# xhuan8/SoccerPlayerShapePose

Hardware: NVIDIA B200
Metric: SMPL meshes/sec fwd+bwd (higher is better)
Workload: dtype f32 (bf16x3 split on tcgen05, fp32 accumulate)

## Files before the change

### soccerplayershapepose_b200/csrc/api.cu

```cuda
#include <atomic>
#include <cstring>
#include <map>
#include <mutex>

#include <nvtx3/nvToolsExt.h>

#include "common.cuh"
#include "umma_common.cuh"

namespace b200smpl {

bool pdl_enabled() {
  static const bool on = getenv("B200_PDL") == nullptr || atoi(getenv("B200_PDL")) != 0;
  return on;
}

NvtxRange::NvtxRange(const char* name) { nvtxRangePushA(name); }
NvtxRange::~NvtxRange() { nvtxRangePop(); }

static thread_local std::string g_last_error;
static std::atomic<long long> g_launches{0};

void set_error(const std::string& msg) { g_last_error = msg; }
int fail(int code, const std::string& msg) {
  g_last_error = msg;
  return code;
}
void count_launch(int n) { g_launches.fetch_add(n, std::memory_order_relaxed); }

static std::atomic<int> g_timing{0};
static std::mutex g_timing_mu;
struct TimingRec { const char* name; cudaEvent_t a, b; };
static std::vector<TimingRec> g_timing_recs;

LaunchTimer::LaunchTimer(const char* name, cudaStream_t st) : name_(name), st_(st), nvtx_(name) {
  if (g_timing.load(std::memory_order_relaxed)) {
    if (cudaEventCreate(&start_) == cudaSuccess) cudaEventRecord(start_, st_);
    else start_ = nullptr;
  }
}
LaunchTimer::~LaunchTimer() {
  if (start_ == nullptr) return;
  cudaEvent_t stop = nullptr;
  if (cudaEventCreate(&stop) != cudaSuccess) return;
  cudaEventRecord(stop, st_);
  std::lock_guard<std::mutex> lk(g_timing_mu);
  g_timing_recs.push_back({name_, start_, stop});
}

static int fwd_gemm_mode(int mode) { return mode == B200SMPL_MODE_BF16_FAST ? B200SMPL_MODE_BF16 : mode; }
static int bwd_gemm_mode(int mode) {
  return mode == B200SMPL_MODE_BF16 ? B200SMPL_MODE_FP32 : (mode == B200SMPL_MODE_BF16_FAST ? B200SMPL_MODE_BF16 : mode);
}

constexpr int DEFAULT_SLAB = 4096;
constexpr int MAX_SLAB = 40960;
static_assert(MAX_SLAB == 2 * BM * BS_MAX_WORK, "slab cap = the forward GEMMs' work-list capacity");
constexpr int MIN_SLABS_PER_SPLIT = 4;

struct Plan {
  int S;
  int k_splits;
  size_t off_feat, off_featf, off_A, off_jposed, off_vpT;
  size_t off_dvp_hi, off_dvp_lo, off_dA, off_dtr, off_dJtot, off_dfeat;
  size_t total;
  size_t saved_slab_bytes;
};

static size_t align_up(size_t x, size_t a) { return (x + a - 1) / a * a; }

static Plan make_plan(const b200smpl_model* m, int batch, int mode, int slab_bodies, bool backward) {
  const DevModel& d = m->dm;
  Plan p{};
  const int Bp = round_up(std::max(batch, 1), 128);
  const int S = slab_bodies > 0 ? round_up(std::min(slab_bodies, MAX_SLAB), 128) : DEFAULT_SLAB;
  p.S = std::min(S, Bp);
  size_t off = 0;
  auto take = [&](size_t bytes) {
    const size_t o = off;
    off = align_up(off + bytes, 1024);
    return o;
  };
  const size_t S_ = (size_t)p.S;
  p.off_feat = take(S_ * d.fl.pitch * 2);
  p.off_featf = take(mode == B200SMPL_MODE_FP32_SIMT ? S_ * d.fl.nf_pad * 4 : 0);
  p.off_A = take((size_t)NJ * AELEMS * S_ * 4);
  p.off_jposed = take((size_t)NJ * 3 * S_ * 4);
  p.off_vpT = take((size_t)d.n_pad * S_ * 4);
  p.saved_slab_bytes = align_up((size_t)NJ * AELEMS * S_ * 4, 1024) + align_up((size_t)d.n_pad * S_ * 4, 1024);
  if (backward) {
    const int bmode = bwd_gemm_mode(mode);
    p.k_splits = bmode == B200SMPL_MODE_FP32_SIMT ? 1 : blend_bwd_umma_splits(d, p.S, m->num_sms);
    p.off_dvp_hi = take(S_ * d.n_pad * 2);
    p.off_dvp_lo = take(bmode == B200SMPL_MODE_BF16 ? 0 : S_ * d.n_pad * 2);
    p.off_dA = take((size_t)(NJ * AELEMS + 3) * S_ * 4);
    p.off_dtr = p.off_dA + (size_t)NJ * AELEMS * S_ * 4;
    p.off_dJtot = take((size_t)std::max(batch, 1) * d.njout * 3 * 4);
    p.off_dfeat = take((size_t)p.k_splits * S_ * d.fl.nf_pad * 4);
  }
  p.total = off + 1024;
  return p;
}

static int check_common(const b200smpl_model* m, int batch, int mode, const void* ws) {
  if (m == nullptr) return fail(B200SMPL_ERR_INVALID, "null model handle");
  if (m->device < 0) return fail(B200SMPL_ERR_CUDA, "host-only model handle: no CUDA device (there is no CPU fallback)");
  if (batch < 1) return fail(B200SMPL_ERR_INVALID, "batch must be >= 1");
  if (mode != B200SMPL_MODE_FP32 && mode != B200SMPL_MODE_BF16 && mode != B200SMPL_MODE_FP32_SIMT &&
      mode != B200SMPL_MODE_BF16_FAST)
    return fail(B200SMPL_ERR_INVALID, "unknown mode");
  if (ws == nullptr) return fail(B200SMPL_ERR_WORKSPACE, "null workspace");
  return 0;
}

}

using namespace b200smpl;

extern "C" {

int b200smpl_abi_version(void) { return B200SMPL_ABI_VERSION; }
const char* b200smpl_last_error(void) { return g_last_error.c_str(); }
int64_t b200smpl_launch_count(void) { return (int64_t)g_launches.load(); }

void b200smpl_timing_enable(int enable) { g_timing.store(enable ? 1 : 0); }

size_t b200smpl_timing_report(char* buf, size_t cap) {
  std::vector<TimingRec> recs;
  {
    std::lock_guard<std::mutex> lk(g_timing_mu);
    recs.swap(g_timing_recs);
  }
  std::map<std::string, std::pair<long long, double>> agg;
  for (auto& r : recs) {
    float ms = 0.f;
    if (cudaEventSynchronize(r.b) == cudaSuccess && cudaEventElapsedTime(&ms, r.a, r.b) == cudaSuccess) {
      auto& e = agg[r.name];
      e.first += 1;
      e.second += ms;
    }
    cudaEventDestroy(r.a);
    cudaEventDestroy(r.b);
  }
  std::string out;
  for (auto& kv : agg) out += kv.first + " " + std::to_string(kv.second.first) + " " + std::to_string(kv.second.second) + "\n";
  if (buf != nullptr && cap > 0) {
    const size_t n = std::min(cap - 1, out.size());
    memcpy(buf, out.data(), n);
    buf[n] = 0;
  }
  return out.size() + 1;
}

int b200smpl_model_create(const b200smpl_model_desc* desc, int device, b200smpl_model** out) {
  B200_NVTX("b200smpl_model_create");
  if (desc == nullptr || out == nullptr) return fail(B200SMPL_ERR_INVALID, "null argument");
  *out = nullptr;
  b200smpl_model* m = new b200smpl_model();
  std::string err;
  int rc = pack_model(desc, m->host, m->dm, err);
  if (rc != 0) {
    delete m;
    return fail(rc, err);
  }
  m->nvj = desc->num_vertex_joints;
  m->nreg = desc->num_regressed_joints;
  m->device = device;
  if (device < 0) {
    *out = m;
    return 0;
  }
  auto cleanup = [&]() {
    for (void* p : m->allocs) cudaFree(p);
    delete m;
  };
  int prev = 0;
  cudaError_t e = cudaGetDevice(&prev);
  if (e == cudaSuccess) e = cudaSetDevice(device);
  if (e != cudaSuccess) {
    cleanup();
    return fail(B200SMPL_ERR_CUDA, std::string("cudaSetDevice: ") + cudaGetErrorString(e));
  }
  cudaDeviceProp prop;
  if (cudaGetDeviceProperties(&prop, device) == cudaSuccess) {
    m->num_sms = prop.multiProcessorCount;
    if (prop.major != 10) {
      cleanup();
      cudaSetDevice(prev);
      return fail(B200SMPL_ERR_CUDA, "this library is built for sm_100a (B200) only; device is sm_" +
                                         std::to_string(prop.major) + std::to_string(prop.minor));
    }
  }
  auto upload = [&](const void* src, size_t bytes, const void** dst) -> bool {
    void* p = nullptr;
    if (cudaMalloc(&p, std::max<size_t>(bytes, 16)) != cudaSuccess) return false;
    m->allocs.push_back(p);
    if (bytes && cudaMemcpy(p, src, bytes, cudaMemcpyHostToDevice) != cudaSuccess) return false;
    *dst = p;
    return true;
  };
  HostArrays& h = m->host;
  DevModel& d = m->dm;
  bool ok = true;
#define UP(field, vec) ok = ok && upload((vec).data(), (vec).size() * sizeof((vec)[0]), (const void**)&d.field)
  UP(Wf, h.Wf);
  UP(Wb_hi, h.Wb_hi);
  UP(Wb_lo, h.Wb_lo);
  UP(W32, h.W32);
  UP(vmeta, h.vmeta);
  UP(vwts, h.vwts);
  UP(vplan, h.vplan);
  UP(Jt, h.Jt);
  UP(Jsd, h.Jsd);
  UP(term_ptr, h.term_ptr);
  UP(term_joint, h.term_joint);
  UP(term_qrow, h.term_qrow);
  UP(term_c, h.term_c);
  UP(qmeta, h.qmeta);
  UP(qcoef, h.qcoef);
  UP(vt_j0, h.vt_j0);
  UP(vt_nj, h.vt_nj);
#undef UP
  cudaSetDevice(prev);
  if (!ok) {
    e = cudaGetLastError();
    cleanup();
    return fail(B200SMPL_ERR_CUDA, std::string("model upload failed: ") + cudaGetErrorString(e));
  }
  *out = m;
  return 0;
}

void b200smpl_model_destroy(b200smpl_model* m) {
  if (m == nullptr) return;
  for (void* p : m->allocs) cudaFree(p);
  delete m;
}

int b200smpl_model_get_info(const b200smpl_model* m, b200smpl_model_info* info) {
  if (m == nullptr || info == nullptr) return fail(B200SMPL_ERR_INVALID, "null argument");
  info->num_verts = m->dm.V;
  info->num_joints_out = m->dm.njout;
  info->num_betas = m->dm.fl.nb;
  info->num_blend_rows = m->dm.n_rows;
  info->num_blend_rows_padded = m->dm.n_pad;
  info->feature_pitch = m->dm.fl.pitch;
  info->num_virtual_groups = m->dm.nq;
  info->device = m->device;
  return 0;
}

int b200smpl_model_debug_array(const b200smpl_model* m, const char* name, const void** data, size_t* bytes) {
  if (m == nullptr || name == nullptr || data == nullptr || bytes == nullptr)
    return fail(B200SMPL_ERR_INVALID, "null argument");
  const HostArrays& h = m->host;
  const std::string n(name);
#define RET(key, vec)                          \
  if (n == key) {                              \
    *data = (vec).data();                      \
    *bytes = (vec).size() * sizeof((vec)[0]);  \
    return 0;                                  \
  }
  RET("Wf", h.Wf) RET("Wb_hi", h.Wb_hi) RET("Wb_lo", h.Wb_lo) RET("W32", h.W32) RET("vmeta", h.vmeta)
  RET("vwts", h.vwts) RET("term_ptr", h.term_ptr) RET("term_joint", h.term_joint) RET("term_qrow", h.term_qrow)
  RET("term_c", h.term_c) RET("Jt", h.Jt) RET("Jsd", h.Jsd) RET("qmeta", h.qmeta) RET("qcoef", h.qcoef)
  RET("vt_j0", h.vt_j0) RET("vt_nj", h.vt_nj) RET("chain_order", h.chain_order) RET("chain_level_ptr", h.chain_level_ptr)
#undef RET
  return fail(B200SMPL_ERR_INVALID, "unknown debug array: " + n);
}

size_t b200smpl_saved_bytes(const b200smpl_model* m, int batch, int slab_bodies) {
  if (m == nullptr) return 0;
  const Plan p = make_plan(m, batch, B200SMPL_MODE_FP32, slab_bodies, false);
  const size_t nslabs = ((size_t)std::max(batch, 1) + p.S - 1) / p.S;
  return nslabs * p.saved_slab_bytes + 1024;
}
size_t b200smpl_forward_workspace_bytes(const b200smpl_model* m, int batch, int mode, int slab_bodies) {
  if (m == nullptr) return 0;
  return make_plan(m, batch, mode, slab_bodies, false).total;
}
size_t b200smpl_backward_workspace_bytes(const b200smpl_model* m, int batch, int mode, int slab_bodies) {
  if (m == nullptr) return 0;
  return make_plan(m, batch, mode, slab_bodies, true).total;
}

int b200smpl_forward(const b200smpl_model* m, const b200smpl_forward_args* a, void* stream) {
  B200_NVTX("b200smpl_forward");
  if (a == nullptr) return fail(B200SMPL_ERR_INVALID, "null args");
  int rc = check_common(m, a->batch, a->mode, a->workspace);
  if (rc) return rc;
  if (!a->betas || !a->pose || !a->joints) return fail(B200SMPL_ERR_INVALID, "betas, pose and joints are required");
  if (a->joints2d && !a->cam) return fail(B200SMPL_ERR_INVALID, "joints2d requires cam");
  const Plan p = make_plan(m, a->batch, a->mode, a->slab_bodies, false);
  if (a->workspace_bytes < p.total) return fail(B200SMPL_ERR_WORKSPACE, "forward workspace too small");
  cudaStream_t st = (cudaStream_t)stream;
  const DevModel& d = m->dm;
  char* ws = (char*)align_up((size_t)a->workspace, 1024);
  __nv_bfloat16* feat = (__nv_bfloat16*)(ws + p.off_feat);
  float* featf = a->mode == B200SMPL_MODE_FP32_SIMT ? (float*)(ws + p.off_featf) : nullptr;
  float* A_T = (float*)(ws + p.off_A);
  float* vpT = (float*)(ws + p.off_vpT);
  const int S = p.S, B = a->batch;
  const bool aa = a->pose_is_axis_angle != 0;
  const int row_begin = a->vertices ? 0 : d.n_virt0;
  char* saved = nullptr;
  if (a->saved) {
    if (a->saved_bytes < b200smpl_saved_bytes(m, B, a->slab_bodies)) return fail(B200SMPL_ERR_WORKSPACE, "saved buffer too small");
    saved = (char*)align_up((size_t)a->saved, 1024);
  }
  for (int b0 = 0; b0 < B; b0 += S) {
    const int nb = std::min(S, B - b0);
    const int Sw = round_up(nb, 128);
    if (saved) {
      A_T = (float*)(saved + (size_t)(b0 / S) * p.saved_slab_bytes);
      vpT = (float*)((char*)A_T + align_up((size_t)NJ * AELEMS * S * 4, 1024));
    }
    if ((rc = launch_pose_fwd(d, a->betas, a->pose, aa, b0, nb, S, Sw, feat, featf, A_T, a->transl, a->joints, st)))
      return rc;
    const bool fused = a->vertices != nullptr && a->mode != B200SMPL_MODE_FP32_SIMT && saved == nullptr && nb >= 512;
    if (fused) {
      rc = launch_blend_lbs_fwd(d, fwd_gemm_mode(a->mode), feat, S, Sw, vpT, A_T, b0, nb, a->transl, a->vertices,
                                m->num_sms, st);
    } else if (a->mode == B200SMPL_MODE_FP32_SIMT) {
      rc = launch_blend_fwd_simt(d, featf, S, Sw, vpT, row_begin, d.n_pad, st);
    } else {
      rc = launch_blend_fwd_umma(d, fwd_gemm_mode(a->mode), feat, S, Sw, vpT, row_begin, d.n_pad, m->num_sms, st);
    }
    if (rc) return rc;
    if (a->vertices && !fused)
      if ((rc = launch_lbs_fwd(d, vpT, S, A_T, b0, nb, a->transl, a->vertices, m->num_sms, st))) return rc;
    if ((rc = launch_joints_fwd(d, vpT, S, A_T, b0, nb, a->transl, a->joints, a->vertices != nullptr && !fused, st))) return rc;
  }
  if (a->joints2d)
    if ((rc = b200smpl_orthographic_project(a->joints, a->cam, a->joints2d, B, d.njout, 0.f, stream))) return rc;
  return 0;
}

int b200smpl_backward(const b200smpl_model* m, const b200smpl_backward_args* a, void* stream) {
  B200_NVTX("b200smpl_backward");
  if (a == nullptr) return fail(B200SMPL_ERR_INVALID, "null args");
  int rc = check_common(m, a->batch, a->mode, a->workspace);
  if (rc) return rc;
  if (!a->betas || !a->pose || !a->grad_betas || !a->grad_pose)
    return fail(B200SMPL_ERR_INVALID, "betas, pose, grad_betas and grad_pose are required");
  if (a->grad_joints2d && (!a->cam || !a->joints))
    return fail(B200SMPL_ERR_INVALID, "grad_joints2d requires cam and the forward joints");
  const Plan p = make_plan(m, a->batch, a->mode, a->slab_bodies, true);
  if (a->workspace_bytes < p.total) return fail(B200SMPL_ERR_WORKSPACE, "backward workspace too small");
  cudaStream_t st = (cudaStream_t)stream;
  const DevModel& d = m->dm;
  const int S = p.S, B = a->batch, nbeta = d.fl.nb;
  const bool aa = a->pose_is_axis_angle != 0;
  const bool have_v = a->grad_vertices != nullptr;
  const bool have_j = a->grad_joints != nullptr || a->grad_joints2d != nullptr;
  if (a->grad_cam && !a->grad_joints2d) B200_CUDA_TRY(cudaMemsetAsync(a->grad_cam, 0, (size_t)B * 3 * 4, st));
  if (!have_v && !have_j) {
    B200_CUDA_TRY(cudaMemsetAsync(a->grad_betas, 0, (size_t)B * nbeta * 4, st));
    B200_CUDA_TRY(cudaMemsetAsync(a->grad_pose, 0, (size_t)B * (aa ? 72 : 216) * 4, st));
    if (a->grad_transl) B200_CUDA_TRY(cudaMemsetAsync(a->grad_transl, 0, (size_t)B * 3 * 4, st));
    return 0;
  }
  char* ws = (char*)align_up((size_t)a->workspace, 1024);
  __nv_bfloat16* feat = (__nv_bfloat16*)(ws + p.off_feat);
  float* featf = a->mode == B200SMPL_MODE_FP32_SIMT ? (float*)(ws + p.off_featf) : nullptr;
  float* A_T = (float*)(ws + p.off_A);
  float* vpT = (float*)(ws + p.off_vpT);
  __nv_bfloat16* dvp_hi = (__nv_bfloat16*)(ws + p.off_dvp_hi);
  const int bmode = bwd_gemm_mode(a->mode);
  __nv_bfloat16* dvp_lo = bmode == B200SMPL_MODE_BF16 ? nullptr : (__nv_bfloat16*)(ws + p.off_dvp_lo);
  float* dA_part = (float*)(ws + p.off_dA);
  float* dtr_part = (float*)(ws + p.off_dtr);
  float* dJtot = (float*)(ws + p.off_dJtot);
  float* dfeat_part = (float*)(ws + p.off_dfeat);
  const float* dJ = a->grad_joints;
  if (a->grad_joints2d) {
    if ((rc = launch_joint_grad_total(a->joints, a->cam, a->grad_joints, a->grad_joints2d, dJtot, a->grad_cam, B,
                                      d.njout, st)))
      return rc;
    dJ = dJtot;
  }
  const int row_begin = have_v ? 0 : d.n_virt0;
  const int row_end = have_j ? d.n_rows : d.n_virt0;
  int k_splits = 1;
  if (a->mode != B200SMPL_MODE_FP32_SIMT) {
    const int slabs = (row_end + 63) / 64 - row_begin / 64;
    k_splits = std::max(1, std::min(p.k_splits, slabs / MIN_SLABS_PER_SPLIT));
  }
  const char* saved = nullptr;
  if (a->saved) {
    if (a->saved_bytes < b200smpl_saved_bytes(m, B, a->slab_bodies)) return fail(B200SMPL_ERR_WORKSPACE, "saved buffer too small");
    saved = (const char*)align_up((size_t)a->saved, 1024);
  }
  for (int b0 = 0; b0 < B; b0 += S) {
    const int nb = std::min(S, B - b0);
    const int Sw = round_up(nb, 128);
    B200_CUDA_TRY(cudaMemsetAsync(dA_part, 0, (size_t)(NJ * AELEMS + 3) * S * 4, st));
    if (saved) {
      A_T = (float*)(saved + (size_t)(b0 / S) * p.saved_slab_bytes);
      vpT = (float*)((char*)A_T + align_up((size_t)NJ * AELEMS * S * 4, 1024));
    } else {
      if ((rc = launch_pose_fwd(d, a->betas, a->pose, aa, b0, nb, S, Sw, feat, featf, A_T, nullptr, nullptr, st)))
        return rc;
      if (a->mode == B200SMPL_MODE_FP32_SIMT)
        rc = launch_blend_fwd_simt(d, featf, S, Sw, vpT, row_begin, d.n_pad, st);
      else
        rc = launch_blend_fwd_umma(d, fwd_gemm_mode(a->mode), feat, S, Sw, vpT, row_begin, d.n_pad, m->num_sms, st);
      if (rc) return rc;
    }
    {
      const size_t c0 = (size_t)row_end / 8, c1 = (size_t)round_up(row_end, 64) / 8;
      if (c1 > c0) {
        const size_t pitch = (size_t)(d.n_pad / 8) * 2048, width = (c1 - c0) * 2048;
        B200_CUDA_TRY(cudaMemset2DAsync(dvp_hi + c0 * 1024, pitch, 0, width, (size_t)Sw / 128, st));
        if (dvp_lo) B200_CUDA_TRY(cudaMemset2DAsync(dvp_lo + c0 * 1024, pitch, 0, width, (size_t)Sw / 128, st));
      }
    }
    if (have_v)
      if ((rc = launch_lbs_bwd(d, vpT, S, Sw, A_T, b0, nb, a->grad_vertices, dvp_hi, dvp_lo, dA_part, dtr_part,
                               m->num_sms, st)))
        return rc;
    if (have_j)
      if ((rc = launch_joints_bwd(d, vpT, S, Sw, A_T, b0, nb, dJ, dvp_hi, dvp_lo, dA_part, dtr_part, have_v, st))) return rc;
    if (a->mode == B200SMPL_MODE_FP32_SIMT)
      rc = launch_blend_bwd_simt(d, dvp_hi, dvp_lo, S, Sw, dfeat_part, row_begin, row_end, st);
    else
      rc = launch_blend_bwd_umma(d, bmode, dvp_hi, dvp_lo, S, Sw, dfeat_part, k_splits, row_begin, row_end, st);
    if (rc) return rc;
    if ((rc = launch_pose_bwd(d, a->betas, a->pose, aa, b0, nb, S, A_T, dA_part, 1, dtr_part, dfeat_part, k_splits,
                              have_j ? dJ : nullptr, a->grad_betas, a->grad_pose, a->grad_transl, st)))
      return rc;
  }
  return 0;
}

}
```

### soccerplayershapepose_b200/csrc/blend_umma.cu

```cuda
#include <cuda.h>
#include <algorithm>

#include "umma_common.cuh"

namespace b200smpl {

template <int BN>
__global__ void __launch_bounds__(GEMM_THREADS, 1)
umma_gemm2_kernel(const __grid_constant__ GemmOps ops, int split3, int ntiles, int nc8, int slab_begin, int slab_end,
                  int slabs_per_split, float* __restrict__ D, int ldd, long long split_stride) {
  constexpr int BNH = BN / 2;
  constexpr int A_BYTES = BM * BK * 2, B_BYTES = BNH * BK * 2;
  static_assert(B_BYTES % 1024 == 0, "the 128-byte swizzle needs every stage offset 1024-byte aligned");
  constexpr int MAX_STAGES = 6;
  constexpr uint32_t TMEM_COLS = 256;
  const int stage_bytes = (split3 ? 2 : 1) * (A_BYTES + B_BYTES);
  const int nstages = split3 ? 3 : 6;
  extern __shared__ unsigned char smem_dyn[];
  unsigned char* smem = reinterpret_cast<unsigned char*>((reinterpret_cast<uintptr_t>(smem_dyn) + 1023) & ~(uintptr_t)1023);
  uint64_t* full_bar = reinterpret_cast<uint64_t*>(smem + MAX_STAGES * (A_BYTES + B_BYTES));
  uint64_t* peer_full_bar = full_bar + MAX_STAGES;
  uint64_t* empty_bar = peer_full_bar + MAX_STAGES;
  uint64_t* tmem_full_bar = empty_bar + MAX_STAGES;
  uint32_t* tmem_slot = reinterpret_cast<uint32_t*>(tmem_full_bar + 1);

  const int warp = threadIdx.x >> 5, lane = threadIdx.x & 31;
  const uint32_t rank = cluster_ctarank();
  const bool padding = (int)blockIdx.x >= ntiles;
  const int m0 = blockIdx.x * BM;
  const int s_begin = slab_begin + blockIdx.z * slabs_per_split;
  const int s_end = min(slab_end, s_begin + slabs_per_split);
  const int total_iters = max(0, s_end - s_begin);

  if (warp == 0 && lane == 0) {
    prefetch_tmap(&ops.wb_hi);
    if (split3) prefetch_tmap(&ops.wb_lo);
  }
  if (warp == 1 && lane == 0) {
    for (int i = 0; i < MAX_STAGES; ++i) {
      mbar_init(&full_bar[i], 1);
      mbar_init(&peer_full_bar[i], 1);
      mbar_init(&empty_bar[i], 1);
    }
    mbar_init(tmem_full_bar, 1);
    fence_barrier_init();
  }
  if (warp == 1) {
    __syncwarp();
    asm volatile("tcgen05.alloc.cta_group::2.sync.aligned.shared::cta.b32 [%0], %1;" ::"r"(smem_u32(tmem_slot)), "r"(TMEM_COLS)
                 : "memory");
    asm volatile("tcgen05.relinquish_alloc_permit.cta_group::2.sync.aligned;" ::: "memory");
  }
  tc_fence_before();
  cluster_sync_all();
  tc_fence_after();
  const uint32_t tmem_base = *tmem_slot;
  pdl_wait();
  if (threadIdx.x == 0) pdl_trigger();
  const int off_bhi = A_BYTES, off_alo = A_BYTES + B_BYTES, off_blo = 2 * A_BYTES + B_BYTES;

  if (warp == 0) {
    const uint64_t pol_stream = l2_policy_evict_first(), pol_keep = l2_policy_evict_last();
    const int tile = padding ? ntiles - 1 : (int)blockIdx.x;
    int stage = 0;
    uint32_t phase = 0;
    for (int it = 0; it < total_iters; ++it) {
      const int slab = s_begin + it;
      mbar_wait(&empty_bar[stage], phase ^ 1);
      unsigned char* sa = smem + stage * stage_bytes;
      if (elect_one()) {
        mbar_arrive_expect_tx(&full_bar[stage], (uint32_t)stage_bytes);
        const size_t aoff = (((size_t)tile * nc8 + (size_t)slab * 8) * 128) * 8;
        bulk_g2s_hint(sa, ops.dvp_hi + aoff, A_BYTES, &full_bar[stage], pol_stream);
        tma_load_2d_hint(sa + off_bhi, &ops.wb_hi, &full_bar[stage], slab * BK, (int)rank * BNH, pol_keep);
        if (split3) {
          bulk_g2s_hint(sa + off_alo, ops.dvp_lo + aoff, A_BYTES, &full_bar[stage], pol_stream);
          tma_load_2d_hint(sa + off_blo, &ops.wb_lo, &full_bar[stage], slab * BK, (int)rank * BNH, pol_keep);
        }
      }
      __syncwarp();
      if (++stage == nstages) { stage = 0; phase ^= 1; }
    }
  } else if (warp == 1) {
    int stage = 0;
    uint32_t phase = 0;
    if (rank == 0) {
      constexpr uint32_t idesc = make_idesc(2 * BM, BN);
      for (int it = 0; it < total_iters; ++it) {
        mbar_wait(&full_bar[stage], phase);
        mbar_wait(&peer_full_bar[stage], phase);
        tc_fence_after();
        const uint32_t sa = smem_u32(smem + stage * stage_bytes);
        const uint64_t da_hi = make_nosw_desc(sa, 2048, 128), db_hi = make_sw128_desc(sa + off_bhi);
        const uint64_t da_lo = make_nosw_desc(sa + off_alo, 2048, 128), db_lo = make_sw128_desc(sa + off_blo);
        if (elect_one()) {
#pragma unroll
          for (int k = 0; k < BK / UMMA_K; ++k)
            umma_bf16_2cta(tmem_base, da_hi + (uint64_t)(k * (4096 >> 4)), db_hi + 2 * k, idesc, (it | k) != 0);
          if (split3) {
#pragma unroll
            for (int k = 0; k < BK / UMMA_K; ++k)
              umma_bf16_2cta(tmem_base, da_lo + (uint64_t)(k * (4096 >> 4)), db_hi + 2 * k, idesc, 1u);
#pragma unroll
            for (int k = 0; k < BK / UMMA_K; ++k)
              umma_bf16_2cta(tmem_base, da_hi + (uint64_t)(k * (4096 >> 4)), db_lo + 2 * k, idesc, 1u);
          }
          umma_commit_2cta(&empty_bar[stage]);
          if (it == total_iters - 1) umma_commit_2cta(tmem_full_bar);
        }
        __syncwarp();
        if (++stage == nstages) { stage = 0; phase ^= 1; }
      }
    } else {
      for (int it = 0; it < total_iters; ++it) {
        mbar_wait(&full_bar[stage], phase);
        if (elect_one()) remote_arrive(&peer_full_bar[stage], 0);
        __syncwarp();
        if (++stage == nstages) { stage = 0; phase ^= 1; }
      }
    }
  } else if (!padding) {
    const int q = warp & 3;
    const int row = m0 + q * 32 + lane;
    float* drow = D + (long long)blockIdx.z * split_stride + (long long)row * ldd;
    if (total_iters > 0) {
      mbar_wait(tmem_full_bar, 0);
      tc_fence_after();
#pragma unroll 1
      for (int c0 = 0; c0 < BN; c0 += 32) {
        uint32_t v[32];
        tmem_ld_32x32(tmem_base + ((uint32_t)(q * 32) << 16) + (uint32_t)c0, v);
        float* o = drow + c0;
#pragma unroll
        for (int i = 0; i < 32; i += 4)
          if (c0 + i < BN)
            *reinterpret_cast<uint4*>(o + i) = make_uint4(v[i], v[i + 1], v[i + 2], v[i + 3]);
      }
    } else {
#pragma unroll 1
      for (int c0 = 0; c0 < BN; c0 += 4) *reinterpret_cast<uint4*>(drow + c0) = make_uint4(0u, 0u, 0u, 0u);
    }
  }
  tc_fence_before();
  cluster_sync_all();
  if (warp == 1) {
    tc_fence_after();
    asm volatile("tcgen05.dealloc.cta_group::2.sync.aligned.b32 %0, %1;" ::"r"(tmem_base), "r"(TMEM_COLS) : "memory");
  }
}

constexpr int WS_STAGES = 5;
constexpr int WS_MAX_SLABS = 9;
constexpr int WS_BN = 128;


template <int DUMMY>
__global__ void __launch_bounds__(GEMM_THREADS, 1)
blend_fwd_bs2_kernel(const __grid_constant__ CUtensorMap map_w, const __grid_constant__ CUtensorMap map_f, int pslabs,
                     int ksteps_cs, int ksteps_p, int use_lo, int row0, int mtiles, int ntiles_n,
                     const __grid_constant__ BsWork work, float4* __restrict__ vpB, int nc4) {
  constexpr int SLAB = BM * BK * 2;
  constexpr int KS = BK / UMMA_K;
  constexpr uint32_t TMEM_COLS = 512;
  const int nslab_f = 1 + 2 * pslabs;
  const int nslab_w = 1 + (use_lo ? 2 : 1) * pslabs;
  extern __shared__ unsigned char smem_dyn[];
  unsigned char* smem = reinterpret_cast<unsigned char*>((reinterpret_cast<uintptr_t>(smem_dyn) + 1023) & ~(uintptr_t)1023);
  unsigned char* f_s = smem;
  unsigned char* w_s = smem + WS_MAX_SLABS * SLAB;
  uint64_t* bars = reinterpret_cast<uint64_t*>(w_s + WS_STAGES * SLAB);
  uint64_t* f_full = bars;
  uint64_t* peer_f_full = bars + 1;
  uint64_t* full_bar = bars + 2;
  uint64_t* peer_full_bar = full_bar + WS_STAGES;
  uint64_t* empty_bar = peer_full_bar + WS_STAGES;
  uint64_t* tfull_bar = empty_bar + WS_STAGES;
  uint64_t* tempty_bar = tfull_bar + 2;
  uint32_t* tmem_slot = reinterpret_cast<uint32_t*>(tempty_bar + 2);

  const int warp = threadIdx.x >> 5, lane = threadIdx.x & 31;
  const uint32_t rank = cluster_ctarank();
  const int piece = (int)(blockIdx.x >> 1);
  const int btile = (int)work.bp[piece] * 2 + (int)rank;
  const int wtp_begin = work.w0[piece], wtp_end = work.w1[piece];

  if (warp == 0 && lane == 0) {
    prefetch_tmap(&map_w);
    prefetch_tmap(&map_f);
  }
  if (warp == 1 && lane == 0) {
    mbar_init(f_full, 1);
    mbar_init(peer_f_full, 1);
    for (int i = 0; i < WS_STAGES; ++i) {
      mbar_init(&full_bar[i], 1);
      mbar_init(&peer_full_bar[i], 1);
      mbar_init(&empty_bar[i], 1);
    }
    for (int i = 0; i < 2; ++i) {
      mbar_init(&tfull_bar[i], 1);
      mbar_init(&tempty_bar[i], 8);
    }
    fence_barrier_init();
  }
  if (warp == 1) {
    __syncwarp();
    asm volatile("tcgen05.alloc.cta_group::2.sync.aligned.shared::cta.b32 [%0], %1;" ::"r"(smem_u32(tmem_slot)), "r"(TMEM_COLS)
                 : "memory");
    asm volatile("tcgen05.relinquish_alloc_permit.cta_group::2.sync.aligned;" ::: "memory");
  }
  tc_fence_before();
  cluster_sync_all();
  tc_fence_after();
  const uint32_t tmem_base = *tmem_slot;
  pdl_wait();
  if (threadIdx.x == 0) pdl_trigger();

  if (warp == 0) {
    if (elect_one()) {
      mbar_arrive_expect_tx(f_full, (uint32_t)nslab_f * SLAB);
      for (int s = 0; s < nslab_f; ++s) tma_load_2d(f_s + s * SLAB, &map_f, f_full, s * BK, btile * WS_BN);
    }
    __syncwarp();
    const uint64_t pol_keep = l2_policy_evict_last();
    int stage = 0;
    uint32_t phase = 0;
    for (int wtp = wtp_begin; wtp < wtp_end; ++wtp)
      for (int s = 0; s < nslab_w; ++s) {
        mbar_wait(&empty_bar[stage], phase ^ 1);
        if (elect_one()) {
          mbar_arrive_expect_tx(&full_bar[stage], SLAB);
          tma_load_2d_hint(w_s + stage * SLAB, &map_w, &full_bar[stage], s * BK, row0 + (wtp * 2 + (int)rank) * BM, pol_keep);
        }
        __syncwarp();
        if (++stage == WS_STAGES) { stage = 0; phase ^= 1; }
      }
  } else if (warp == 1) {
    int stage = 0;
    uint32_t phase = 0;
    if (rank == 0) {
      constexpr uint32_t idesc = make_idesc(2 * BM, 2 * WS_BN);
      mbar_wait(f_full, 0);
      mbar_wait(peer_f_full, 0);
      uint32_t tph0 = 0, tph1 = 0;
      int acc = 0;
      for (int wtp = wtp_begin; wtp < wtp_end; ++wtp, acc ^= 1) {
        const uint32_t tph = acc ? tph1 : tph0;
        mbar_wait(&tempty_bar[acc], tph ^ 1);
        if (acc) tph1 ^= 1; else tph0 ^= 1;
        tc_fence_after();
        const uint32_t d_tmem = tmem_base + (uint32_t)(acc * 2 * WS_BN);
        for (int s = 0; s < nslab_w; ++s) {
          mbar_wait(&full_bar[stage], phase);
          mbar_wait(&peer_full_bar[stage], phase);
          tc_fence_after();
          const uint64_t db = make_sw128_desc(smem_u32(w_s + stage * SLAB));
          int ks = ksteps_cs, f0 = 0, f1 = -1;
          if (s > 0) {
            const int j = (s - 1) % pslabs;
            ks = min(KS, ksteps_p - j * KS);
            f0 = 1 + j;
            if (s <= pslabs) f1 = 1 + pslabs + j;
          }
          const uint64_t da0 = make_sw128_desc(smem_u32(f_s + f0 * SLAB));
          const uint64_t da1 = make_sw128_desc(smem_u32(f_s + max(f1, 0) * SLAB));
          if (elect_one()) {
#pragma unroll
            for (int k = 0; k < KS; ++k)
              if (k < ks) umma_bf16_2cta(d_tmem, da0 + 2 * k, db + 2 * k, idesc, (s | k) != 0);
            if (f1 >= 0) {
#pragma unroll
              for (int k = 0; k < KS; ++k)
                if (k < ks) umma_bf16_2cta(d_tmem, da1 + 2 * k, db + 2 * k, idesc, 1u);
            }
            umma_commit_2cta(&empty_bar[stage]);
            if (s == nslab_w - 1) umma_commit_2cta(&tfull_bar[acc]);
          }
          __syncwarp();
          if (++stage == WS_STAGES) { stage = 0; phase ^= 1; }
        }
      }
    } else {
      mbar_wait(f_full, 0);
      if (elect_one()) remote_arrive(peer_f_full, 0);
      __syncwarp();
      for (int wtp = wtp_begin; wtp < wtp_end; ++wtp)
        for (int s = 0; s < nslab_w; ++s) {
          mbar_wait(&full_bar[stage], phase);
          if (elect_one()) remote_arrive(&peer_full_bar[stage], 0);
          __syncwarp();
          if (++stage == WS_STAGES) { stage = 0; phase ^= 1; }
        }
    }
  } else {
    const int q = warp & 3;
    uint32_t tph0 = 0, tph1 = 0;
    int acc = 0;
    for (int wtp = wtp_begin; wtp < wtp_end; ++wtp, acc ^= 1) {
      const uint32_t tph = acc ? tph1 : tph0;
      mbar_wait(&tfull_bar[acc], tph);
      if (acc) tph1 ^= 1; else tph0 ^= 1;
      tc_fence_after();
      if (btile < ntiles_n) {
        const bool live_hi = wtp * 2 + 1 < mtiles;
        float4* colbase = vpB + ((size_t)(btile * 4 + q) * nc4 + ((row0 + wtp * 2 * BM) >> 2)) * 32 + lane;
#pragma unroll 1
        for (int c0 = 0; c0 < 2 * WS_BN; c0 += 32) {
          if (c0 >= WS_BN && !live_hi) continue;
          uint32_t v[32];
          tmem_ld_32x32(tmem_base + ((uint32_t)(q * 32) << 16) + (uint32_t)(acc * 2 * WS_BN + c0), v);
          float4* o = colbase + (size_t)(c0 >> 2) * 32;
#pragma unroll
          for (int i = 0; i < 8; ++i)
            o[i * 32] = make_float4(__uint_as_float(v[4 * i]), __uint_as_float(v[4 * i + 1]),
                                    __uint_as_float(v[4 * i + 2]), __uint_as_float(v[4 * i + 3]));
        }
      }
      tc_fence_before();
      __syncwarp();
      if (lane == 0) {
        if (rank == 0) asm volatile("mbarrier.arrive.shared::cta.b64 _, [%0];" ::"r"(smem_u32(&tempty_bar[acc])) : "memory");
        else remote_arrive(&tempty_bar[acc], 0);
      }
    }
  }
  tc_fence_before();
  cluster_sync_all();
  if (warp == 1) {
    tc_fence_after();
    asm volatile("tcgen05.dealloc.cta_group::2.sync.aligned.b32 %0, %1;" ::"r"(tmem_base), "r"(TMEM_COLS) : "memory");
  }
}

typedef CUresult (*EncodeTiledFn)(CUtensorMap*, CUtensorMapDataType, cuuint32_t, void*, const cuuint64_t*,
                                  const cuuint64_t*, const cuuint32_t*, const cuuint32_t*, CUtensorMapInterleave,
                                  CUtensorMapSwizzle, CUtensorMapL2promotion, CUtensorMapFloatOOBfill);

static EncodeTiledFn get_encode_fn() {
  static EncodeTiledFn fn = nullptr;
  if (fn == nullptr) {
    void* p = nullptr;
    cudaDriverEntryPointQueryResult qres;
    if (cudaGetDriverEntryPoint("cuTensorMapEncodeTiled", &p, cudaEnableDefault, &qres) == cudaSuccess &&
        qres == cudaDriverEntryPointSuccess)
      fn = reinterpret_cast<EncodeTiledFn>(p);
  }
  return fn;
}

int make_map(CUtensorMap* map, const void* base, int k_extent, int rows, int pitch_elems, int box_rows) {
  EncodeTiledFn fn = get_encode_fn();
  if (fn == nullptr) return fail(B200SMPL_ERR_CUDA, "cuTensorMapEncodeTiled entry point not available");
  cuuint64_t dims[2] = {(cuuint64_t)k_extent, (cuuint64_t)rows};
  cuuint64_t strides[1] = {(cuuint64_t)pitch_elems * 2};
  cuuint32_t box[2] = {(cuuint32_t)BK, (cuuint32_t)box_rows};
  cuuint32_t estr[2] = {1, 1};
  CUresult r = fn(map, CU_TENSOR_MAP_DATA_TYPE_BFLOAT16, 2, const_cast<void*>(base), dims, strides, box, estr,
                  CU_TENSOR_MAP_INTERLEAVE_NONE, CU_TENSOR_MAP_SWIZZLE_128B, CU_TENSOR_MAP_L2_PROMOTION_L2_256B,
                  CU_TENSOR_MAP_FLOAT_OOB_FILL_NONE);
  if (r != CUDA_SUCCESS) return fail(B200SMPL_ERR_CUDA, "cuTensorMapEncodeTiled failed with code " + std::to_string((int)r));
  return 0;
}

int build_bs_work(int bp_total, int wtp_total, int tpcs, BsWork& work) {
  if (bp_total < 1 || wtp_total < 1) return -1;
  const long long total = (long long)bp_total * wtp_total;
  const int nranges = (int)std::min<long long>(total, std::max(tpcs, bp_total));
  struct Piece { int bp, w0, w1; };
  std::vector<Piece> pieces;
  for (int r = 0; r < nranges; ++r) {
    long long lo = total * r / nranges, hi = total * (r + 1) / nranges;
    while (lo < hi) {
      const int bp = (int)(lo / wtp_total);
      const long long end = std::min<long long>(hi, (long long)(bp + 1) * wtp_total);
      pieces.push_back({bp, (int)(lo - (long long)bp * wtp_total), (int)(end - (long long)bp * wtp_total)});
      lo = end;
    }
  }
  const int rect_chunks = std::max(1, std::min(wtp_total, tpcs / std::max(1, bp_total)));
  const int rect_len = (wtp_total + rect_chunks - 1) / rect_chunks;
  const int flat_len = (int)((total + nranges - 1) / nranges);
  if ((int)pieces.size() > BS_MAX_WORK || rect_len <= flat_len + 1) {
    pieces.clear();
    const int chunks = std::max(1, std::min(rect_chunks, BS_MAX_WORK / bp_total));
    const int wpc = (wtp_total + chunks - 1) / chunks;
    for (int bp = 0; bp < bp_total; ++bp)
      for (int w = 0; w < wtp_total; w += wpc) pieces.push_back({bp, w, std::min(wtp_total, w + wpc)});
    if ((int)pieces.size() > BS_MAX_WORK) return -1;
  }
  std::stable_sort(pieces.begin(), pieces.end(), [](const Piece& a, const Piece& b) { return a.w1 - a.w0 > b.w1 - b.w0; });
  memset(&work, 0, sizeof(work));
  int npieces = 0;
  for (const Piece& pc : pieces) {
    work.bp[npieces] = (uint16_t)pc.bp; work.w0[npieces] = (uint16_t)pc.w0; work.w1[npieces] = (uint16_t)pc.w1;
    ++npieces;
  }
  return npieces;
}

int launch_blend_fwd_umma(const DevModel& m, int mode, const __nv_bfloat16* feat, int S, int Sw, float* vpT,
                          int row_begin, int row_end, int num_sms, cudaStream_t st) {
  const int pslabs = m.fl.pseg / BK;
  const int use_lo = (mode == B200SMPL_MODE_BF16) ? 0 : 1;
  if (1 + 2 * pslabs > WS_MAX_SLABS) return fail(B200SMPL_ERR_INVALID, "feature pitch too large for the resident operand");
  CUtensorMap map_w, map_f;
  int rc;
  if ((rc = make_map(&map_w, m.Wf, m.fl.pitch, m.n_pad, m.fl.pitch, BM))) return rc;
  if ((rc = make_map(&map_f, feat, m.fl.pitch, Sw, m.fl.pitch, WS_BN))) return rc;
  constexpr int smem = (WS_MAX_SLABS + WS_STAGES) * BM * BK * 2 + 1024 + 256;
  auto kern = blend_fwd_bs2_kernel<0>;
  B200_SMEM_ATTR_ONCE(kern, smem);
  const int mtiles = (row_end - row_begin) / BM;
  const int wtp_total = (mtiles + 1) / 2;
  const int ntiles_n = Sw / WS_BN;
  const int bp_total = (ntiles_n + 1) / 2;
  BsWork work;
  const int npieces = build_bs_work(bp_total, wtp_total, std::max(1, num_sms / 2), work);
  if (npieces < 0) return fail(B200SMPL_ERR_INVALID, "slab too wide for the forward GEMM work list");
  cudaLaunchConfig_t cfg;
  memset(&cfg, 0, sizeof(cfg));
  cfg.gridDim = dim3(2 * npieces, 1, 1);
  cfg.blockDim = dim3(GEMM_THREADS, 1, 1);
  cfg.dynamicSmemBytes = smem;
  cfg.stream = st;
  cudaLaunchAttribute attr[2];
  attr[0].id = cudaLaunchAttributeClusterDimension;
  attr[0].val.clusterDim.x = 2;
  attr[0].val.clusterDim.y = 1;
  attr[0].val.clusterDim.z = 1;
  attr[1].id = cudaLaunchAttributeProgrammaticStreamSerialization;
  attr[1].val.programmaticStreamSerializationAllowed = 1;
  cfg.attrs = attr;
  cfg.numAttrs = pdl_enabled() ? 2 : 1;
  LaunchTimer _timer("blend_fwd_umma", st);
  B200_CUDA_TRY(cudaLaunchKernelEx(&cfg, kern, map_w, map_f, pslabs, (m.fl.k_cs + UMMA_K - 1) / UMMA_K,
                                   (NPOSE + UMMA_K - 1) / UMMA_K, use_lo, row_begin, mtiles, ntiles_n, work,
                                   reinterpret_cast<float4*>(vpT), m.n_pad / 4));
  B200_LAUNCH_CHECK("blend_fwd_umma");
  return 0;
}

}
extern "C" int b200smpl_debug_fwd_gemm_worklist(int body_tiles, int row_tiles, int num_sms, uint16_t* out, int capacity) {
  using namespace b200smpl;
  BsWork work;
  const int n = build_bs_work((body_tiles + 1) / 2, (row_tiles + 1) / 2, std::max(1, num_sms / 2), work);
  if (n < 0 || out == nullptr || n > capacity) return n < 0 ? -1 : n;
  for (int c = 0; c < n; ++c) { out[c * 3] = work.bp[c]; out[c * 3 + 1] = work.w0[c]; out[c * 3 + 2] = work.w1[c]; }
  return n;
}
namespace b200smpl {

int blend_bwd_umma_splits(const DevModel& m, int S, int num_sms) {
  const int mtiles = round_up((S + BM - 1) / BM, 2);
  const int slabs = (m.n_rows + BK - 1) / BK;
  int want = std::max(1, num_sms / mtiles);
  want = std::max(1, std::min(want, slabs / 8));
  return want;
}

template <int BN>
static int launch_bwd_pair(const GemmOps& ops, int split3, int ntiles, int nc8, int slab_begin, int slab_end,
                           int nsplit, float* dfeat_part, long long split_stride, cudaStream_t st) {
  constexpr int smem = 6 * (BM * BK * 2 + (BN / 2) * BK * 2) + 1024 + 512;
  auto kern = umma_gemm2_kernel<BN>;
  B200_SMEM_ATTR_ONCE(kern, smem);
  const int slabs = slab_end - slab_begin;
  const int sps = (slabs + nsplit - 1) / nsplit;
  cudaLaunchConfig_t cfg;
  memset(&cfg, 0, sizeof(cfg));
  cfg.gridDim = dim3(round_up(ntiles, 2), 1, nsplit);
  cfg.blockDim = dim3(GEMM_THREADS, 1, 1);
  cfg.dynamicSmemBytes = smem;
  cfg.stream = st;
  cudaLaunchAttribute attr[2];
  attr[0].id = cudaLaunchAttributeClusterDimension;
  attr[0].val.clusterDim.x = 2;
  attr[0].val.clusterDim.y = 1;
  attr[0].val.clusterDim.z = 1;
  attr[1].id = cudaLaunchAttributeProgrammaticStreamSerialization;
  attr[1].val.programmaticStreamSerializationAllowed = 1;
  cfg.attrs = attr;
  cfg.numAttrs = pdl_enabled() ? 2 : 1;
  LaunchTimer _timer("blend_bwd_umma", st);
  B200_CUDA_TRY(cudaLaunchKernelEx(&cfg, kern, ops, split3, ntiles, nc8, slab_begin, slab_end, sps, dfeat_part, BN,
                                   split_stride));
  B200_LAUNCH_CHECK("blend_bwd_umma");
  return 0;
}

int launch_blend_bwd_umma(const DevModel& m, int mode, const __nv_bfloat16* dvp_hi, const __nv_bfloat16* dvp_lo,
                          int S, int Sw, float* dfeat_part, int nsplit, int row_begin, int row_end,
                          cudaStream_t st) {
  const int nf_pad = m.fl.nf_pad;
  if (nf_pad != 208 && nf_pad != 224)
    return fail(B200SMPL_ERR_INVALID, "unsupported num_betas for the tensor-core backward (nf_pad=" + std::to_string(nf_pad) + ")");
  const bool split3 = (mode != B200SMPL_MODE_BF16) && dvp_lo != nullptr;
  GemmOps ops;
  memset(&ops, 0, sizeof(ops));
  ops.dvp_hi = dvp_hi;
  ops.dvp_lo = dvp_lo;
  int rc;
  if ((rc = make_map(&ops.wb_hi, m.Wb_hi, row_end, nf_pad, m.n_pad, nf_pad / 2))) return rc;
  if (split3 && (rc = make_map(&ops.wb_lo, m.Wb_lo, row_end, nf_pad, m.n_pad, nf_pad / 2))) return rc;
  const int slab_begin = row_begin / BK, slab_end = (row_end + BK - 1) / BK;
  const long long split_stride = (long long)S * nf_pad;
  auto launch = nf_pad == 224 ? launch_bwd_pair<224> : launch_bwd_pair<208>;
  return launch(ops, split3 ? 1 : 0, Sw / BM, m.n_pad / 8, slab_begin, slab_end, nsplit, dfeat_part, split_stride, st);
}

}
```

### soccerplayershapepose_b200/csrc/common.cuh

```cuda
#pragma once

#include <cuda_bf16.h>
#include <cuda_runtime.h>
#include <stdint.h>

#include <cstring>
#include <string>
#include <utility>
#include <vector>

#include "../../include/b200smpl.h"

namespace b200smpl {

constexpr int NJ = 24;
constexpr int NPOSE = 9 * (NJ - 1);
constexpr int AELEMS = 12;
constexpr int TILE_V = 32;
constexpr int MAX_CHILD = 4;
constexpr int MAX_BETAS = 16;

constexpr uint32_t VMETA_VALID = 1u << 29;

struct ChainTables {
  int8_t parent[NJ];
  int8_t depth[NJ];
  int8_t nchild[NJ];
  int8_t child[NJ][MAX_CHILD];
  int8_t maxchild_at[NJ];
  int8_t order[NJ];
  int8_t level_ptr[NJ + 1];
  int32_t maxdepth;
};

struct FeatLayout {
  int nb;
  int off_s0, off_s1, off_s2;
  int k_cs;
  int pseg;
  int off_p0;
  int off_p1;
  int pitch;
  int nf;
  int nf_pad;
};

inline int round_up(int x, int m) { return (x + m - 1) / m * m; }

inline FeatLayout make_feat_layout(int nb) {
  FeatLayout L;
  L.nb = nb;
  L.off_s0 = 3;
  L.off_s1 = 3 + nb;
  L.off_s2 = 3 + 2 * nb;
  L.k_cs = 3 + 3 * nb;
  L.pseg = round_up(NPOSE, 64);
  L.off_p0 = 64;
  L.off_p1 = 64 + L.pseg;
  L.pitch = 64 + 2 * L.pseg;
  L.nf = nb + NPOSE;
  L.nf_pad = round_up(L.nf, 16);
  return L;
}

struct DevModel {
  int V;
  int ntiles;
  int n_real;
  int nq;
  int n_rows;
  int n_virt0;
  int n_pad;
  int njout;
  int nterms;
  int ntv;
  int vt_maxcols;
  FeatLayout fl;
  ChainTables chain;
  const __nv_bfloat16* Wf;
  const __nv_bfloat16* Wb_hi;
  const __nv_bfloat16* Wb_lo;
  const float* W32;
  const uint32_t* vmeta;
  const float4* vwts;
  const uint32_t* vplan;
  const float* Jt;
  const float* Jsd;
  const int32_t* term_ptr;
  const uint8_t* term_joint;
  const int32_t* term_qrow;
  const float* term_c;
  const uint32_t* qmeta;
  const float* qcoef;
  const int32_t* vt_j0;
  const int32_t* vt_nj;
};

struct HostArrays {
  std::vector<__nv_bfloat16> Wf, Wb_hi, Wb_lo;
  std::vector<float> W32, Jt, Jsd, term_c;
  std::vector<uint32_t> vmeta;
  std::vector<float> vwts;
  std::vector<uint32_t> vplan;
  std::vector<int32_t> term_ptr, term_qrow, vt_j0, vt_nj;
  std::vector<int8_t> chain_order, chain_level_ptr;
  std::vector<uint32_t> qmeta;
  std::vector<float> qcoef;
  std::vector<uint8_t> term_joint;
};

}

struct b200smpl_model {
  int device = -1;
  b200smpl::DevModel dm{};
  b200smpl::HostArrays host;
  std::vector<void*> allocs;
  int nvj = 0, nreg = 0;
  int num_sms = 148;
};

namespace b200smpl {

void set_error(const std::string& msg);
int fail(int code, const std::string& msg);
void count_launch(int n = 1);

struct NvtxRange {
  explicit NvtxRange(const char* name);
  ~NvtxRange();
};
#define B200_NVTX(name) ::b200smpl::NvtxRange _nvtx_range(name)

struct LaunchTimer {
  LaunchTimer(const char* name, cudaStream_t st);
  ~LaunchTimer();
  const char* name_;
  cudaStream_t st_;
  cudaEvent_t start_ = nullptr;
  NvtxRange nvtx_;
};

bool pdl_enabled();
#ifdef __CUDACC__
__device__ __forceinline__ void pdl_wait() { asm volatile("griddepcontrol.wait;" ::: "memory"); }
__device__ __forceinline__ void pdl_trigger() { asm volatile("griddepcontrol.launch_dependents;" ::: "memory"); }

template <typename... KArgs, typename... Args>
inline cudaError_t launch_k(void (*kern)(KArgs...), dim3 grid, dim3 block, size_t smem, cudaStream_t st, bool pdl,
                            Args&&... args) {
  cudaLaunchConfig_t cfg;
  memset(&cfg, 0, sizeof(cfg));
  cfg.gridDim = grid;
  cfg.blockDim = block;
  cfg.dynamicSmemBytes = smem;
  cfg.stream = st;
  cudaLaunchAttribute attr[1];
  attr[0].id = cudaLaunchAttributeProgrammaticStreamSerialization;
  attr[0].val.programmaticStreamSerializationAllowed = 1;
  cfg.attrs = attr;
  cfg.numAttrs = (pdl && pdl_enabled()) ? 1 : 0;
  return cudaLaunchKernelEx(&cfg, kern, static_cast<KArgs>(std::forward<Args>(args))...);
}
#endif

#define B200_SMEM_ATTR_ONCE(kern, bytes)                                                          \
  do {                                                                                            \
    static int _granted[64] = {};                                                                 \
    int _dev = 0;                                                                                 \
    B200_CUDA_TRY(cudaGetDevice(&_dev));                                                          \
    if (_dev < 0 || _dev >= 64 || (int)(bytes) > _granted[_dev]) {                                \
      B200_CUDA_TRY(cudaFuncSetAttribute(kern, cudaFuncAttributeMaxDynamicSharedMemorySize, (int)(bytes))); \
      if (_dev >= 0 && _dev < 64) _granted[_dev] = (int)(bytes);                                  \
    }                                                                                             \
  } while (0)

#define B200_CUDA_TRY(expr)                                                                       \
  do {                                                                                            \
    cudaError_t _e = (expr);                                                                      \
    if (_e != cudaSuccess)                                                                        \
      return ::b200smpl::fail(B200SMPL_ERR_CUDA, std::string(#expr) + ": " + cudaGetErrorString(_e)); \
  } while (0)

#define B200_LAUNCH_CHECK(name)                                                                   \
  do {                                                                                            \
    cudaError_t _e = cudaGetLastError();                                                          \
    if (_e != cudaSuccess)                                                                        \
      return ::b200smpl::fail(B200SMPL_ERR_CUDA, std::string("launch ") + name + ": " + cudaGetErrorString(_e)); \
    ::b200smpl::count_launch();                                                                   \
  } while (0)

int pack_model(const b200smpl_model_desc* d, HostArrays& h, DevModel& dm, std::string& err);

int launch_pose_fwd(const DevModel& m, const float* betas, const float* pose, bool axis_angle, int b0, int nb, int S,
                    int Sw, __nv_bfloat16* feat, float* featf, float* A_blk, const float* transl, float* joints,
                    cudaStream_t st);
int launch_pose_bwd(const DevModel& m, const float* betas, const float* pose, bool axis_angle, int b0, int nb, int S,
                    const float* A_blk, const float* dA_part, int n_dA_parts, const float* dtr_part, const float* dfeat_part,
                    int n_dfeat_parts, const float* dJ, float* grad_betas, float* grad_pose,
                    float* grad_transl, cudaStream_t st);

int launch_blend_fwd_simt(const DevModel& m, const float* featf, int S, int Sw, float* vpT, int row_begin,
                          int row_end, cudaStream_t st);
int launch_blend_bwd_simt(const DevModel& m, const __nv_bfloat16* dvp_hi, const __nv_bfloat16* dvp_lo, int S, int Sw,
                          float* dfeat, int row_begin, int row_end, cudaStream_t st);
int launch_blend_fwd_umma(const DevModel& m, int mode, const __nv_bfloat16* feat, int S, int Sw, float* vpT,
                          int row_begin, int row_end, int num_sms, cudaStream_t st);
int launch_blend_bwd_umma(const DevModel& m, int mode, const __nv_bfloat16* dvp_hi, const __nv_bfloat16* dvp_lo,
                          int S, int Sw, float* dfeat_part, int nsplit, int row_begin, int row_end,
                          cudaStream_t st);
int blend_bwd_umma_splits(const DevModel& m, int S, int num_sms);
int launch_blend_lbs_fwd(const DevModel& m, int mode, const __nv_bfloat16* feat, int S, int Sw, float* vpT,
                         const float* A_blk, int b0, int nb, const float* transl, float* verts, int num_sms,
                         cudaStream_t st);

int launch_lbs_fwd(const DevModel& m, const float* vpT, int S, const float* A_T, int b0, int nb,
                   const float* transl, float* verts, int num_sms, cudaStream_t st);
int launch_lbs_bwd(const DevModel& m, const float* vpT, int S, int Sw, const float* A_T, int b0, int nb,
                   const float* grad_verts, __nv_bfloat16* dvp_hi, __nv_bfloat16* dvp_lo, float* dA_acc,
                   float* dtr_acc, int num_sms, cudaStream_t st);

int launch_joints_fwd(const DevModel& m, const float* vpB, int S, const float* A_blk, int b0, int nb,
                      const float* transl, float* joints, bool after_lbs, cudaStream_t st);
int launch_joints_bwd(const DevModel& m, const float* vpB, int S, int Sw, const float* A_blk, int b0, int nb,
                      const float* dJ, __nv_bfloat16* dvp_hi, __nv_bfloat16* dvp_lo, float* dA_part, float* dtr_part,
                      bool after_lbs, cudaStream_t st);
int launch_joint_grad_total(const float* joints, const float* cam, const float* gj, const float* g2d, float* dJ,
                            float* gcam, int B, int nj, cudaStream_t st);

}
```

### soccerplayershapepose_b200/csrc/fused_fwd.cu

```cuda
#include <algorithm>

#include "lbs_tiles.cuh"
#include "umma_common.cuh"

namespace b200smpl {

constexpr int FF_BN = 96;
constexpr int FF_BNH = FF_BN / 2;
constexpr int FF_NW = 2;
constexpr int FF_STAGES = 7;
constexpr int FF_STAGE_BYTES = FF_BNH * BK * 2;
constexpr int FF_PS = (NPOSE + BK - 1) / BK;
constexpr int FF_KSP = (NPOSE + UMMA_K - 1) / UMMA_K;
constexpr int FF_MAX_SLABS = 1 + 2 * FF_PS;
constexpr int FF_SLAB = BM * BK * 2;
constexpr int FF_EPI_WARPS = 4 * FF_NW;
constexpr int FF_EPI_WARP0 = 2;
constexpr int FF_THREADS = (FF_EPI_WARP0 + FF_EPI_WARPS) * 32;
constexpr int FF_HV = 8;
constexpr int FF_TR_COL = 2 * FF_BN;
constexpr int FF_WV = TILE_V / 2;
constexpr int FF_PLAN_WORDS = (FF_WV / 8) * 40;
constexpr int FF_TILE_WORDS = ItemShape<FF_HV>::TILE_WORDS;
constexpr int FF_NBARS = 1 + 2 * FF_STAGES + 4 + 2 * FF_EPI_WARPS;
constexpr size_t FF_SMEM = (size_t)FF_MAX_SLABS * FF_SLAB + (size_t)FF_STAGES * FF_STAGE_BYTES +
                           (size_t)FF_EPI_WARPS * (FF_TILE_WORDS + 2 * FF_PLAN_WORDS) * 4 + FF_NBARS * 8 + 16 +
                           1024 ;
static_assert(FF_SMEM <= 232448, "fused forward: shared memory budget");
static_assert(FF_TR_COL + NJ * AELEMS <= 512, "fused forward: tensor memory budget");
static_assert(NJ % FF_NW == 0, "joints split evenly over the warps of a quadrant");

__device__ __forceinline__ void tma_load_2d_pair(void* smem_dst, const CUtensorMap* map, uint64_t* bar, int c0, int c1,
                                                 uint64_t policy) {
  asm volatile(
      "cp.async.bulk.tensor.2d.cta_group::2.shared::cluster.global.mbarrier::complete_tx::bytes.L2::cache_hint [%0], [%1, {%3, %4}], [%2], %5;"
      ::"r"(smem_u32(smem_dst)), "l"(map), "r"(smem_u32(bar) & 0xFEFFFFFFu), "r"(c0), "r"(c1), "l"(policy)
      : "memory");
}

__device__ __forceinline__ void tmem_st_x4(uint32_t taddr, const float4& v) {
  asm volatile("tcgen05.st.sync.aligned.32x32b.x4.b32 [%0], {%1, %2, %3, %4};"
               ::"r"(taddr), "r"(__float_as_uint(v.x)), "r"(__float_as_uint(v.y)), "r"(__float_as_uint(v.z)),
                 "r"(__float_as_uint(v.w))
               : "memory");
}
__device__ __forceinline__ void tmem_wait_st() { asm volatile("tcgen05.wait::st.sync.aligned;" ::: "memory"); }
__device__ __forceinline__ void tmem_ld_12(uint32_t taddr, uint32_t (&r)[12]) {
  asm volatile(
      "tcgen05.ld.sync.aligned.32x32b.x4.b32 {%0, %1, %2, %3}, [%12];\n\t"
      "tcgen05.ld.sync.aligned.32x32b.x4.b32 {%4, %5, %6, %7}, [%13];\n\t"
      "tcgen05.ld.sync.aligned.32x32b.x4.b32 {%8, %9, %10, %11}, [%14];\n\t"
      "tcgen05.wait::ld.sync.aligned;"
      : "=r"(r[0]), "=r"(r[1]), "=r"(r[2]), "=r"(r[3]), "=r"(r[4]), "=r"(r[5]), "=r"(r[6]), "=r"(r[7]), "=r"(r[8]),
        "=r"(r[9]), "=r"(r[10]), "=r"(r[11])
      : "r"(taddr), "r"(taddr + 4), "r"(taddr + 8)
      : "memory");
}
__device__ __forceinline__ void tmem_ld_24(uint32_t taddr, uint32_t (&r)[24]) {
  asm volatile(
      "tcgen05.ld.sync.aligned.32x32b.x8.b32 {%0, %1, %2, %3, %4, %5, %6, %7}, [%24];\n\t"
      "tcgen05.ld.sync.aligned.32x32b.x8.b32 {%8, %9, %10, %11, %12, %13, %14, %15}, [%25];\n\t"
      "tcgen05.ld.sync.aligned.32x32b.x8.b32 {%16, %17, %18, %19, %20, %21, %22, %23}, [%26];\n\t"
      "tcgen05.wait::ld.sync.aligned;"
      : "=r"(r[0]), "=r"(r[1]), "=r"(r[2]), "=r"(r[3]), "=r"(r[4]), "=r"(r[5]), "=r"(r[6]), "=r"(r[7]), "=r"(r[8]),
        "=r"(r[9]), "=r"(r[10]), "=r"(r[11]), "=r"(r[12]), "=r"(r[13]), "=r"(r[14]), "=r"(r[15]), "=r"(r[16]),
        "=r"(r[17]), "=r"(r[18]), "=r"(r[19]), "=r"(r[20]), "=r"(r[21]), "=r"(r[22]), "=r"(r[23])
      : "r"(taddr), "r"(taddr + 8), "r"(taddr + 16)
      : "memory");
}

template <bool HI>
__device__ __forceinline__ void load_slot_tm(SlotXY& s, SlotZ2& z, uint32_t tr_base, int joint) {
  uint32_t r[12];
  tmem_ld_12(tr_base + (uint32_t)(joint * AELEMS), r);
  s.c0 = mk2(__uint_as_float(r[0]), __uint_as_float(r[1]));
  s.c1 = mk2(__uint_as_float(r[2]), __uint_as_float(r[3]));
  s.c2 = mk2(__uint_as_float(r[4]), __uint_as_float(r[5]));
  s.t = mk2(__uint_as_float(r[6]), __uint_as_float(r[7]));
  z.r20 = set_half<HI>(z.r20, __uint_as_float(r[8]));
  z.r21 = set_half<HI>(z.r21, __uint_as_float(r[9]));
  z.r22 = set_half<HI>(z.r22, __uint_as_float(r[10]));
  z.t2 = set_half<HI>(z.t2, __uint_as_float(r[11]));
}

__device__ __forceinline__ void skin_fwd4_tm(Slots& s, uint32_t tr_base, const uint32_t* meta_s, const float4* wts_s,
                                             uint32_t force, float tx, float ty, float tz, const float (&P)[12],
                                             float* row_out) {
  const uint4 m4 = *reinterpret_cast<const uint4*>(meta_s);
  const uint32_t mts[4] = {m4.x | force, m4.y, m4.z, m4.w};
  float4 ws[4];
#pragma unroll
  for (int i = 0; i < 4; ++i) ws[i] = wts_s[i];
  float o[12];
  const f2 txy = mk2(tx, ty), tz0 = mk2(tz, 0.f);
#pragma unroll
  for (int i = 0; i < 4; ++i) {
    const uint32_t mt = mts[i];
    const float4 w = ws[i];
    if (mt & (0xFu << 20)) {
      if (mt & (1u << 20)) load_slot_tm<false>(s.s0, s.zA, tr_base, mt & 31);
      if (mt & (1u << 21)) load_slot_tm<true>(s.s1, s.zA, tr_base, (mt >> 5) & 31);
      if (mt & (1u << 22)) load_slot_tm<false>(s.s2, s.zB, tr_base, (mt >> 10) & 31);
      if (mt & (1u << 23)) load_slot_tm<true>(s.s3, s.zB, tr_base, (mt >> 15) & 31);
    }
    const f2 px = bc2(P[i * 3]), py = bc2(P[i * 3 + 1]), pz = bc2(P[i * 3 + 2]);
    f2 oxy = txy;
#define B200_SKIN_XY(sl, wk) oxy = fma2(bc2(wk), fma2(sl.c0, px, fma2(sl.c1, py, fma2(sl.c2, pz, sl.t))), oxy);
    B200_SKIN_XY(s.s0, w.x)
    B200_SKIN_XY(s.s1, w.y)
    B200_SKIN_XY(s.s2, w.z)
    B200_SKIN_XY(s.s3, w.w)
#undef B200_SKIN_XY
    f2 oz = fma2(mk2(w.x, w.y), fma2(s.zA.r20, px, fma2(s.zA.r21, py, fma2(s.zA.r22, pz, s.zA.t2))), tz0);
    oz = fma2(mk2(w.z, w.w), fma2(s.zB.r20, px, fma2(s.zB.r21, py, fma2(s.zB.r22, pz, s.zB.t2))), oz);
    o[i * 3] = lo2(oxy); o[i * 3 + 1] = hi2(oxy); o[i * 3 + 2] = lo2(oz) + hi2(oz);
  }
#pragma unroll
  for (int i = 0; i < 3; ++i)
    *reinterpret_cast<float4*>(row_out + i * 4) = make_float4(o[i * 4], o[i * 4 + 1], o[i * 4 + 2], o[i * 4 + 3]);
}

template <bool USE_LO>
__global__ void __launch_bounds__(FF_THREADS, 1)
blend_lbs_fwd_kernel(const __grid_constant__ CUtensorMap map_w, const __grid_constant__ CUtensorMap map_f,
                     int ksteps_cs, int n_pad, int ntiles_n,
                     const __grid_constant__ BsWork work, float4* __restrict__ vpB, int nc4,
                     const float4* __restrict__ A_blk, int b0, int nb, const float* __restrict__ transl,
                     float* __restrict__ verts, int V, int n_vtiles, int vec_ok, const uint32_t* __restrict__ vplan) {
  constexpr int KS = BK / UMMA_K;
  constexpr uint32_t TMEM_COLS = 512;
  using SH = ItemShape<FF_HV>;
  constexpr int PS = FF_PS;
  constexpr int nslab_f = 1 + 2 * PS;
  constexpr int nslab_w = 1 + (USE_LO ? 2 : 1) * PS;
  extern __shared__ __align__(1024) unsigned char smem_dyn[];
  unsigned char* smem = smem_dyn + ((1024u - (smem_u32(smem_dyn) & 1023u)) & 1023u);
  unsigned char* f_s = smem;
  unsigned char* w_s = f_s + FF_MAX_SLABS * FF_SLAB;
  float* tiles = reinterpret_cast<float*>(w_s + FF_STAGES * FF_STAGE_BYTES);
  uint32_t* stashes = reinterpret_cast<uint32_t*>(tiles + FF_EPI_WARPS * FF_TILE_WORDS);
  uint64_t* bars = reinterpret_cast<uint64_t*>(stashes + FF_EPI_WARPS * 2 * FF_PLAN_WORDS);
  uint64_t* f_full = bars;
  uint64_t* full_bar = bars + 1;
  uint64_t* empty_bar = full_bar + FF_STAGES;
  uint64_t* tfull_bar = empty_bar + FF_STAGES;
  uint64_t* tempty_bar = tfull_bar + 2;
  uint64_t* wbars = tempty_bar + 2;
  uint32_t* tmem_slot = reinterpret_cast<uint32_t*>(wbars + 2 * FF_EPI_WARPS);

  const int warp = threadIdx.x >> 5, lane = threadIdx.x & 31;
  const uint32_t rank = cluster_ctarank();
  const int piece = (int)(blockIdx.x >> 1);
  const int btile = (int)work.bp[piece] * 2 + (int)rank;
  const int wt_begin = work.w0[piece], wt_end = work.w1[piece];

  if (warp == 0 && lane == 0) {
    prefetch_tmap(&map_w);
    prefetch_tmap(&map_f);
  }
  if (warp == 1 && lane == 0) {
    mbar_init(f_full, 1);
    for (int i = 0; i < FF_STAGES; ++i) {
      mbar_init(&full_bar[i], 1);
      mbar_init(&empty_bar[i], 1);
    }
    for (int i = 0; i < 2; ++i) {
      mbar_init(&tfull_bar[i], 1);
      mbar_init(&tempty_bar[i], 16);
    }
    for (int i = 0; i < 2 * FF_EPI_WARPS; ++i) mbar_init(&wbars[i], 1);
    fence_barrier_init();
  }
  if (warp == 1) {
    __syncwarp();
    asm volatile("tcgen05.alloc.cta_group::2.sync.aligned.shared::cta.b32 [%0], %1;" ::"r"(smem_u32(tmem_slot)), "r"(TMEM_COLS)
                 : "memory");
    asm volatile("tcgen05.relinquish_alloc_permit.cta_group::2.sync.aligned;" ::: "memory");
  }
  tc_fence_before();
  cluster_sync_all();
  tc_fence_after();
  const uint32_t tmem_base = *tmem_slot;
  pdl_wait();
  if (threadIdx.x == 0) pdl_trigger();

  if (warp < FF_EPI_WARP0) {
  if (warp == 0) {
    const uint64_t pol_keep = l2_policy_evict_last();
    if (elect_one()) {
      if (rank == 0) mbar_arrive_expect_tx(f_full, 2u * (uint32_t)nslab_f * FF_SLAB);
      for (int s = 0; s < nslab_f; ++s) tma_load_2d_pair(f_s + s * FF_SLAB, &map_f, f_full, s * BK, btile * BM, l2_policy_evict_first());
    }
    __syncwarp();
    int stage = 0;
    uint32_t phase = 0;
    for (int wt = wt_begin; wt < wt_end; ++wt)
      for (int s = 0; s < nslab_w; ++s) {
        mbar_wait(&empty_bar[stage], phase ^ 1);
        if (elect_one()) {
          if (rank == 0) mbar_arrive_expect_tx(&full_bar[stage], 2 * FF_STAGE_BYTES);
          tma_load_2d_pair(w_s + stage * FF_STAGE_BYTES, &map_w, &full_bar[stage], s * BK, wt * FF_BN + (int)rank * FF_BNH, pol_keep);
        }
        __syncwarp();
        if (++stage == FF_STAGES) { stage = 0; phase ^= 1; }
      }
  } else if (warp == 1) {
    int stage = 0;
    uint32_t phase = 0;
    if (rank == 0) {
      constexpr uint32_t idesc = make_idesc(2 * BM, FF_BN);
      mbar_wait(f_full, 0);
      const uint64_t da_base = make_sw128_desc(smem_u32(f_s));
      const uint64_t db_base = make_sw128_desc(smem_u32(w_s));
      uint32_t tph0 = 0, tph1 = 0;
      int acc = 0;
      auto slab = [&](uint32_t d_tmem, int ks, int f0, int f1, bool first, uint64_t* tfull) {
        mbar_wait(&full_bar[stage], phase);
        tc_fence_after();
        const uint64_t db = db_base + (uint64_t)(stage * (FF_STAGE_BYTES >> 4));
        if (elect_one()) {
          const uint64_t da0 = da_base + (uint64_t)(f0 * (FF_SLAB >> 4));
#pragma unroll
          for (int k = 0; k < KS; ++k)
            if (k < ks) umma_bf16_2cta(d_tmem, da0 + 2 * k, db + 2 * k, idesc, (first && k == 0) ? 0u : 1u);
          if (f1 >= 0) {
            const uint64_t da1 = da_base + (uint64_t)(f1 * (FF_SLAB >> 4));
#pragma unroll
            for (int k = 0; k < KS; ++k)
              if (k < ks) umma_bf16_2cta(d_tmem, da1 + 2 * k, db + 2 * k, idesc, 1u);
          }
          umma_commit_2cta(&empty_bar[stage]);
          if (tfull != nullptr) umma_commit_2cta(tfull);
        }
        __syncwarp();
        if (++stage == FF_STAGES) { stage = 0; phase ^= 1; }
      };
#pragma unroll 1
      for (int wt = wt_begin; wt < wt_end; ++wt, acc ^= 1) {
        const uint32_t tph = acc ? tph1 : tph0;
        mbar_wait(&tempty_bar[acc], tph ^ 1);
        if (acc) tph1 ^= 1; else tph0 ^= 1;
        tc_fence_after();
        const uint32_t d_tmem = tmem_base + (uint32_t)(acc * FF_BN);
        slab(d_tmem, ksteps_cs, 0, -1, true, nullptr);
#pragma unroll
        for (int j = 0; j < PS; ++j)
          slab(d_tmem, min(KS, FF_KSP - j * KS), 1 + j, 1 + PS + j, false, (!USE_LO && j == PS - 1) ? &tfull_bar[acc] : nullptr);
        if (USE_LO) {
#pragma unroll
          for (int j = 0; j < PS; ++j)
            slab(d_tmem, min(KS, FF_KSP - j * KS), 1 + j, -1, false, j == PS - 1 ? &tfull_bar[acc] : nullptr);
        }
      }
    }
  }
  } else {
    const int e = warp - FF_EPI_WARP0, q = warp & 3, r3 = e >> 2;
    float* tile = tiles + e * FF_TILE_WORDS;
    float* my_row = tile + lane * SH::HROW;
    uint32_t* stash = stashes + e * 2 * FF_PLAN_WORDS;
    uint64_t* wbar = wbars + e * 2;
    const bool live = btile < ntiles_n;
    const int g = btile * 4 + q;
    const uint32_t lane_base = tmem_base + ((uint32_t)(q * 32) << 16);
    const uint32_t tr_base = lane_base + FF_TR_COL;
    const bool skin = verts != nullptr;
    if (live && skin) {
      const float4* ap = A_blk + (size_t)g * (NJ * 3 * 32) + lane;
#pragma unroll 1
      for (int j = r3 * (NJ / FF_NW); j < (r3 + 1) * (NJ / FF_NW); ++j) {
        const float4 x0 = ap[(j * 3) * 32], x1 = ap[(j * 3 + 1) * 32], x2 = ap[(j * 3 + 2) * 32];
        tmem_st_x4(tr_base + j * AELEMS, x0);
        tmem_st_x4(tr_base + j * AELEMS + 4, x1);
        tmem_st_x4(tr_base + j * AELEMS + 8, x2);
      }
      tmem_wait_st();
    }
    tc_fence_before();
    asm volatile("bar.sync %0, %1;" ::"r"(1 + q), "n"(32 * FF_NW) : "memory");
    tc_fence_after();
    float tx = 0.f, ty = 0.f, tz = 0.f;
    if (live && transl != nullptr && g * 32 + lane < nb) {
      const float* tp = transl + (size_t)(b0 + g * 32 + lane) * 3;
      tx = tp[0]; ty = tp[1]; tz = tp[2];
    }
    const int nrows = max(0, min(32, nb - g * 32));
    float* v_g = skin ? verts + (size_t)(b0 + g * 32) * V * 3 : nullptr;
    const size_t row_stride = (size_t)V * 3;
    auto release = [&](int acc) {
      tc_fence_before();
      __syncwarp();
      if (lane == 0) {
        if (rank == 0) asm volatile("mbarrier.arrive.shared::cta.b64 _, [%0];" ::"r"(smem_u32(&tempty_bar[acc])) : "memory");
        else remote_arrive(&tempty_bar[acc], 0);
      }
    };
    const int nhalf = 2 * (wt_end - wt_begin);
    auto is_vhalf = [&](int h) { return h < nhalf && wt_begin + (h >> 1) < n_vtiles; };
    auto issue_plan = [&](uint32_t b, int h) {
      mbar_expect_tx(&wbar[b], FF_PLAN_WORDS * 4);
      bulk_g2s(stash + b * FF_PLAN_WORDS, vplan + ((size_t)(wt_begin + (h >> 1)) * 2 + (h & 1)) * FF_PLAN_WORDS,
               FF_PLAN_WORDS * 4, &wbar[b]);
    };
    uint32_t n_plan = 0;
    if (live && skin && is_vhalf(r3) && lane == 0) issue_plan(0u, r3);
    Slots sl;
    sl.zA.r20 = sl.zA.r21 = sl.zA.r22 = sl.zA.t2 = sl.zB.r20 = sl.zB.r21 = sl.zB.r22 = sl.zB.t2 = mk2(0.f, 0.f);
    sl.s0.c0 = sl.s0.c1 = sl.s0.c2 = sl.s0.t = sl.s1.c0 = sl.s1.c1 = sl.s1.c2 = sl.s1.t = mk2(0.f, 0.f);
    sl.s2.c0 = sl.s2.c1 = sl.s2.c2 = sl.s2.t = sl.s3.c0 = sl.s3.c1 = sl.s3.c2 = sl.s3.t = mk2(0.f, 0.f);
#pragma unroll 1
    for (int h = r3; h < nhalf; h += FF_NW) {
      const int ti = h >> 1, half = h & 1, wt = wt_begin + ti, acc = ti & 1;
      mbar_wait(&tfull_bar[acc], (uint32_t)(ti >> 1) & 1u);
      tc_fence_after();
      if (!live) {
        release(acc);
        continue;
      }
      const int row_w = wt * FF_BN + half * (FF_BN / 2);
      const uint32_t acc_base = lane_base + (uint32_t)(acc * FF_BN + half * (FF_BN / 2));
      if (skin && wt < n_vtiles) {
        const uint32_t b = n_plan & 1;
        if (is_vhalf(h + FF_NW) && lane == 0) issue_plan(b ^ 1, h + FF_NW);
        mbar_wait(&wbar[b], (n_plan >> 1) & 1);
        const uint32_t* st = stash + b * FF_PLAN_WORDS;
#pragma unroll 1
        for (int sub = 0; sub < FF_WV / FF_HV; ++sub) {
          uint32_t v[24];
          tmem_ld_24(acc_base + (uint32_t)(sub * 24), v);
          if (sub == FF_WV / FF_HV - 1) release(acc);
#pragma unroll
          for (int u = 0; u < FF_HV / 4; ++u) {
            float P[12];
#pragma unroll
            for (int i = 0; i < 12; ++i)
              P[i] = __uint_as_float(v[u * 12 + i]);
            skin_fwd4_tm(sl, tr_base, plan_meta(st, sub * (FF_HV / 4) + u), plan_wts(st, sub * (FF_HV / 4) + u),
                         (sub == 0 && u == 0) ? (0xFu << 20) : 0u, tx, ty, tz, P, my_row + u * 12);
          }
          __syncwarp();
          {
            const int vbase = wt * TILE_V + half * FF_WV + sub * FF_HV;
            const int ncols = max(0, min(FF_HV, V - vbase)) * 3;
            float* dst0 = v_g + (size_t)vbase * 3;
            if (!vec_ok) tile_to_global_scalar<FF_HV>(tile, dst0, row_stride, nrows, ncols, lane);
            else tile_to_global<FF_HV>(tile, dst0, row_stride, nrows, ncols, lane);
          }
          __syncwarp();
        }
        ++n_plan;
      } else {
        float4* colbase = vpB + ((size_t)g * nc4 + (row_w >> 2)) * 32 + lane;
#pragma unroll 1
        for (int c0 = 0; c0 < FF_BN / 2; c0 += 24) {
          uint32_t v[24];
          tmem_ld_24(acc_base + (uint32_t)c0, v);
          if (c0 + 24 >= FF_BN / 2) release(acc);
          float4* o = colbase + (size_t)(c0 >> 2) * 32;
#pragma unroll
          for (int i = 0; i < 6; ++i)
            if (row_w + c0 + 4 * i < n_pad)
              o[i * 32] = make_float4(__uint_as_float(v[4 * i]), __uint_as_float(v[4 * i + 1]),
                                      __uint_as_float(v[4 * i + 2]), __uint_as_float(v[4 * i + 3]));
        }
      }
    }
  }
  tc_fence_before();
  cluster_sync_all();
  if (warp == 1) {
    tc_fence_after();
    asm volatile("tcgen05.dealloc.cta_group::2.sync.aligned.b32 %0, %1;" ::"r"(tmem_base), "r"(TMEM_COLS) : "memory");
  }
}

int launch_blend_lbs_fwd(const DevModel& m, int mode, const __nv_bfloat16* feat, int S, int Sw, float* vpT,
                         const float* A_blk, int b0, int nb, const float* transl, float* verts, int num_sms,
                         cudaStream_t st) {
  (void)S;
  const bool use_lo = mode != B200SMPL_MODE_BF16;
  if (m.fl.pseg != FF_PS * BK) return fail(B200SMPL_ERR_INVALID, "fused forward: unexpected pose segment width");
  if (m.n_virt0 != m.ntiles * FF_BN) return fail(B200SMPL_ERR_INVALID, "fused forward: vertex tiles must be 96 rows");
  CUtensorMap map_w, map_f;
  int rc;
  if ((rc = make_map(&map_w, m.Wf, m.fl.pitch, m.n_pad, m.fl.pitch, FF_BNH))) return rc;
  if ((rc = make_map(&map_f, feat, m.fl.pitch, Sw, m.fl.pitch, BM))) return rc;
  auto kern = use_lo ? blend_lbs_fwd_kernel<true> : blend_lbs_fwd_kernel<false>;
  B200_SMEM_ATTR_ONCE(blend_lbs_fwd_kernel<true>, FF_SMEM);
  B200_SMEM_ATTR_ONCE(blend_lbs_fwd_kernel<false>, FF_SMEM);
  const int wt_total = (m.n_pad + FF_BN - 1) / FF_BN;
  const int ntiles_n = Sw / BM;
  const int bp_total = (ntiles_n + 1) / 2;
  BsWork work;
  const int npieces = build_bs_work(bp_total, wt_total, std::max(1, num_sms / 2), work);
  if (npieces < 0) return fail(B200SMPL_ERR_INVALID, "slab too wide for the fused forward work list");
  const int vec_ok = (verts != nullptr && (m.V & 1) == 0 && (reinterpret_cast<uintptr_t>(verts) & 7) == 0) ? 1 : 0;
  cudaLaunchConfig_t cfg;
  memset(&cfg, 0, sizeof(cfg));
  cfg.gridDim = dim3(2 * npieces, 1, 1);
  cfg.blockDim = dim3(FF_THREADS, 1, 1);
  cfg.dynamicSmemBytes = FF_SMEM;
  cfg.stream = st;
  cudaLaunchAttribute attr[2];
  attr[0].id = cudaLaunchAttributeClusterDimension;
  attr[0].val.clusterDim.x = 2;
  attr[0].val.clusterDim.y = 1;
  attr[0].val.clusterDim.z = 1;
  attr[1].id = cudaLaunchAttributeProgrammaticStreamSerialization;
  attr[1].val.programmaticStreamSerializationAllowed = 1;
  cfg.attrs = attr;
  cfg.numAttrs = pdl_enabled() ? 2 : 1;
  LaunchTimer _timer("blend_lbs_fwd", st);
  B200_CUDA_TRY(cudaLaunchKernelEx(&cfg, kern, map_w, map_f, (m.fl.k_cs + UMMA_K - 1) / UMMA_K, m.n_pad, ntiles_n, work,
                                   reinterpret_cast<float4*>(vpT), m.n_pad / 4, reinterpret_cast<const float4*>(A_blk), b0, nb,
                                   transl, verts, m.V, m.ntiles, vec_ok, m.vplan));
  B200_LAUNCH_CHECK("blend_lbs_fwd");
  return 0;
}

}
```

### soccerplayershapepose_b200/csrc/joints.cu

```cuda
#include "skin_common.cuh"

namespace b200smpl {

constexpr int JW = 8;
constexpr int JQ = 4;
constexpr int JTL = JW / JQ;
constexpr int JT = JW * 32;

__device__ __forceinline__ void load_q24(float (&q)[24], const float4* __restrict__ p) {
#pragma unroll
  for (int i = 0; i < 6; ++i) {
    const float4 v = ld_stream4(p + i * 32);
    q[i * 4] = v.x; q[i * 4 + 1] = v.y; q[i * 4 + 2] = v.z; q[i * 4 + 3] = v.w;
  }
}
__device__ __forceinline__ void load_slot_s(float (&a)[AELEMS], const float* A_s, int joint, int lane) {
  const float4* p = reinterpret_cast<const float4*>(A_s) + joint * 96 + lane;
  unpack_transform(a, p[0], p[32], p[64]);
}
__device__ __forceinline__ void quartet_sync(int tl) { asm volatile("bar.sync %0, 128;" ::"r"(1 + tl) : "memory"); }

__global__ void __launch_bounds__(JT, 1024 / JT)
joints_fwd_kernel(DevModel m, const float4* __restrict__ vpB, int nc4, const float4* __restrict__ A_blk, int b0, int nb,
                  int pitch, const float* __restrict__ transl, float* __restrict__ joints) {
  extern __shared__ __align__(128) float smem[];
  float* A_s = smem;
  const int warp = threadIdx.x >> 5, lane = threadIdx.x & 31;
  const int tl = warp / JQ, qt = warp % JQ;
  float* my_row = smem + AG_WORDS + warp * 32 * pitch + lane * pitch;
  uint64_t* bar = reinterpret_cast<uint64_t*>(smem + AG_WORDS + JW * 32 * pitch + ((JW * 32 * pitch) & 1));
  const int g = blockIdx.x;
  if (threadIdx.x == 0) fetch_group_transforms(A_s, reinterpret_cast<const float*>(A_blk), g, bar);
  const int tv = blockIdx.y * JTL + tl;
  const bool on = tv < m.ntv;
  float q[24];
  uint32_t mt_l = 0;
  float c_l = 0.f;
  int ncols = 0;
  if (on) {
    load_q24(q, vpB + ((size_t)g * nc4 + (m.ntiles + tv) * 24 + qt * 6) * 32 + lane);
    mt_l = __ldg(m.qmeta + tv * 32 + qt * 8 + (lane & 7));
    c_l = __ldg(m.qcoef + tv * 32 + qt * 8 + (lane & 7));
    float tx = 0.f, ty = 0.f, tz = 0.f;
    if (qt == 0 && transl != nullptr && g * 32 + lane < nb) {
      const float* t = transl + (size_t)(b0 + g * 32 + lane) * 3;
      tx = t[0]; ty = t[1]; tz = t[2];
    }
    ncols = m.vt_nj[tv] * 3;
    for (int c = 0; c < ncols; c += 3) { my_row[c] = tx; my_row[c + 1] = ty; my_row[c + 2] = tz; }
  }
  __syncthreads();
  if (on) {
    mbar_wait(bar, 0);
    float a[AELEMS];
#pragma unroll
    for (int ii = 0; ii < 8; ++ii) {
      const uint32_t mt = __shfl_sync(0xffffffffu, mt_l, ii);
      if (!(mt & (1u << 14))) continue;
      if (ii == 0 || (mt & (1u << 5))) load_slot_s(a, A_s, mt & 31, lane);
      const float c = __shfl_sync(0xffffffffu, c_l, ii);
      const float qx = q[ii * 3], qy = q[ii * 3 + 1], qz = q[ii * 3 + 2];
      float* o = my_row + ((mt >> 8) & 31) * 3;
      o[0] += fmaf(a[0], qx, fmaf(a[1], qy, fmaf(a[2], qz, a[3] * c)));
      o[1] += fmaf(a[4], qx, fmaf(a[5], qy, fmaf(a[6], qz, a[7] * c)));
      o[2] += fmaf(a[8], qx, fmaf(a[9], qy, fmaf(a[10], qz, a[11] * c)));
    }
    quartet_sync(tl);
    const int r = qt * 8 + (lane >> 2);
    if (g * 32 + r < nb) {
      const float* p0 = smem + AG_WORDS + (tl * JQ) * 32 * pitch + r * pitch;
      float* dst = joints + (size_t)(b0 + g * 32 + r) * m.njout * 3 + (size_t)(NJ + m.vt_j0[tv]) * 3;
      for (int c = lane & 3; c < ncols; c += 4)
        dst[c] = (p0[c] + p0[32 * pitch + c]) + (p0[64 * pitch + c] + p0[96 * pitch + c]);
    }
  }
  pdl_wait();
}

__global__ void __launch_bounds__(JT, 768 / JT)
joints_bwd_kernel(DevModel m, const float4* __restrict__ vpB, int nc4, const float4* __restrict__ A_blk, int b0, int nb,
                  int pitch, const float* __restrict__ dJ, __nv_bfloat16* __restrict__ dvp_hi,
                  __nv_bfloat16* __restrict__ dvp_lo, float* __restrict__ dA_acc, float* __restrict__ dtr_acc) {
  extern __shared__ __align__(128) float smem[];
  float* A_s = smem;
  const int warp = threadIdx.x >> 5, lane = threadIdx.x & 31;
  const int tl = warp / JQ, qt = warp % JQ;
  float* tile = smem + AG_WORDS + tl * 32 * pitch;
  const float* my_row = tile + lane * pitch;
  uint64_t* bar = reinterpret_cast<uint64_t*>(smem + AG_WORDS + JTL * 32 * pitch + ((JTL * 32 * pitch) & 1));
  const int g = blockIdx.x;
  if (threadIdx.x == 0) fetch_group_transforms(A_s, reinterpret_cast<const float*>(A_blk), g, bar);
  const int tv = blockIdx.y * JTL + tl;
  const bool on = tv < m.ntv;
  float q[24];
  uint32_t mt_l = 0;
  float c_l = 0.f;
  int ncols = 0;
  if (on) {
    load_q24(q, vpB + ((size_t)g * nc4 + (m.ntiles + tv) * 24 + qt * 6) * 32 + lane);
    mt_l = __ldg(m.qmeta + tv * 32 + qt * 8 + (lane & 7));
    c_l = __ldg(m.qcoef + tv * 32 + qt * 8 + (lane & 7));
    ncols = m.vt_nj[tv] * 3;
    {
      const int r = qt * 8 + (lane >> 2);
      const bool live = g * 32 + r < nb;
      const float* src = dJ + (size_t)(b0 + g * 32 + r) * m.njout * 3 + (size_t)(NJ + m.vt_j0[tv]) * 3;
      float* trow = tile + r * pitch;
      for (int c0 = lane & 3; c0 < ncols; c0 += 16) {
        float v[4];
#pragma unroll
        for (int u = 0; u < 4; ++u) v[u] = (live && c0 + u * 4 < ncols) ? ld_stream(src + c0 + u * 4) : 0.f;
#pragma unroll
        for (int u = 0; u < 4; ++u)
          if (c0 + u * 4 < ncols) trow[c0 + u * 4] = v[u];
      }
    }
  }
  __syncthreads();
  if (on) {
    mbar_wait(bar, 0);
    if (qt == 0) {
      float sx = 0.f, sy = 0.f, sz = 0.f;
      for (int c = 0; c < ncols; c += 3) { sx += my_row[c]; sy += my_row[c + 1]; sz += my_row[c + 2]; }
      float* dtr_g = dtr_acc + (size_t)g * 96;
      red_add(dtr_g + lane, sx);
      red_add(dtr_g + 32 + lane, sy);
      red_add(dtr_g + 64 + lane, sz);
    }
    float* dA_g = dA_acc + (size_t)g * AG_WORDS;
    float a[AELEMS], d[AELEMS], dq[24];
#pragma unroll
    for (int e = 0; e < AELEMS; ++e) d[e] = 0.f;
    int jcur = 0;
#pragma unroll
    for (int ii = 0; ii < 8; ++ii) {
      const uint32_t mt = __shfl_sync(0xffffffffu, mt_l, ii);
      if (!(mt & (1u << 14))) {
        dq[ii * 3] = dq[ii * 3 + 1] = dq[ii * 3 + 2] = 0.f;
        continue;
      }
      if (ii == 0 || (mt & (1u << 5))) {
        if (ii != 0) flush_slot_g(d, dA_g, jcur, lane);
        jcur = mt & 31;
        load_slot_s(a, A_s, jcur, lane);
      }
      const float c = __shfl_sync(0xffffffffu, c_l, ii);
      const float* gj = my_row + ((mt >> 8) & 31) * 3;
      const float gx = gj[0], gy = gj[1], gz = gj[2];
      const float qx = q[ii * 3], qy = q[ii * 3 + 1], qz = q[ii * 3 + 2];
      dq[ii * 3] = fmaf(a[0], gx, fmaf(a[4], gy, a[8] * gz));
      dq[ii * 3 + 1] = fmaf(a[1], gx, fmaf(a[5], gy, a[9] * gz));
      dq[ii * 3 + 2] = fmaf(a[2], gx, fmaf(a[6], gy, a[10] * gz));
      d[0] = fmaf(gx, qx, d[0]); d[1] = fmaf(gx, qy, d[1]); d[2] = fmaf(gx, qz, d[2]); d[3] = fmaf(gx, c, d[3]);
      d[4] = fmaf(gy, qx, d[4]); d[5] = fmaf(gy, qy, d[5]); d[6] = fmaf(gy, qz, d[6]); d[7] = fmaf(gy, c, d[7]);
      d[8] = fmaf(gz, qx, d[8]); d[9] = fmaf(gz, qy, d[9]); d[10] = fmaf(gz, qz, d[10]); d[11] = fmaf(gz, c, d[11]);
    }
    const size_t chunk0 = (size_t)(g >> 2) * (nc4 >> 1) + (size_t)((m.ntiles + tv) * 12 + qt * 3);
    __nv_bfloat16* hi_p = dvp_hi + (chunk0 * 128 + (g & 3) * 32 + lane) * 8;
    __nv_bfloat16* lo_p = dvp_lo ? dvp_lo + (chunk0 * 128 + (g & 3) * 32 + lane) * 8 : nullptr;
#pragma unroll
    for (int cc = 0; cc < 3; ++cc) {
      const float ch[8] = {dq[cc * 8], dq[cc * 8 + 1], dq[cc * 8 + 2], dq[cc * 8 + 3],
                           dq[cc * 8 + 4], dq[cc * 8 + 5], dq[cc * 8 + 6], dq[cc * 8 + 7]};
      const size_t off = (size_t)cc * 128 * 8;
      store_dvp_chunk(ch, hi_p + off, lo_p ? lo_p + off : nullptr);
    }
    if (__shfl_sync(0xffffffffu, mt_l, 0) & (1u << 14)) flush_slot_g(d, dA_g, jcur, lane);
  }
  pdl_wait();
}

__global__ void __launch_bounds__(128)
joint_grad_total_kernel(const float* __restrict__ joints, const float* __restrict__ cam,
                        const float* __restrict__ gj, const float* __restrict__ g2d, float* __restrict__ dJ,
                        float* __restrict__ gcam, int nj) {
  __shared__ float sh[3][4];
  const int b = blockIdx.x;
  const float s = cam[b * 3], tx = cam[b * 3 + 1], ty = cam[b * 3 + 2];
  float gs = 0.f, gtx = 0.f, gty = 0.f;
  for (int j = threadIdx.x; j < nj; j += blockDim.x) {
    const size_t o3 = ((size_t)b * nj + j) * 3, o2 = ((size_t)b * nj + j) * 2;
    const float gu = g2d[o2], gv = g2d[o2 + 1];
    dJ[o3] = (gj ? gj[o3] : 0.f) + s * gu;
    dJ[o3 + 1] = (gj ? gj[o3 + 1] : 0.f) + s * gv;
    dJ[o3 + 2] = gj ? gj[o3 + 2] : 0.f;
    gs += gu * (joints[o3] + tx) + gv * (joints[o3 + 1] + ty);
    gtx += s * gu;
    gty += s * gv;
  }
  float v[3] = {gs, gtx, gty};
#pragma unroll
  for (int k = 0; k < 3; ++k) {
#pragma unroll
    for (int o = 16; o > 0; o >>= 1) v[k] += __shfl_xor_sync(0xffffffffu, v[k], o);
    if ((threadIdx.x & 31) == 0) sh[k][threadIdx.x >> 5] = v[k];
  }
  __syncthreads();
  if (gcam != nullptr && threadIdx.x < 3) gcam[b * 3 + threadIdx.x] = sh[threadIdx.x][0] + sh[threadIdx.x][1] + sh[threadIdx.x][2] + sh[threadIdx.x][3];
}

static int joints_split(int ntv) { return std::max(1, (ntv + JTL - 1) / JTL); }
static size_t joints_smem(int ntiles_s, int pitch) { return (size_t)(AG_WORDS + ntiles_s * 32 * pitch + 1) * 4 + 16; }

int launch_joints_fwd(const DevModel& m, const float* vpB, int S, const float* A_blk, int b0, int nb,
                      const float* transl, float* joints, bool after_lbs, cudaStream_t st) {
  if (nb <= 0 || m.ntv == 0) return 0;
  const int groups = (nb + 31) / 32;
  const int pitch = m.vt_maxcols | 1;
  const size_t smem = joints_smem(JW, pitch);
  B200_SMEM_ATTR_ONCE(joints_fwd_kernel, smem);
  LaunchTimer _timer("joints_fwd", st);
  B200_CUDA_TRY(launch_k(joints_fwd_kernel, dim3(groups, joints_split(m.ntv)), dim3(JT), smem, st, after_lbs, m,
                         reinterpret_cast<const float4*>(vpB), m.n_pad / 4, reinterpret_cast<const float4*>(A_blk), b0, nb, pitch,
                         transl, joints));
  B200_LAUNCH_CHECK("joints_fwd");
  return 0;
}

int launch_joints_bwd(const DevModel& m, const float* vpB, int S, int Sw, const float* A_blk, int b0, int nb,
                      const float* dJ, __nv_bfloat16* dvp_hi, __nv_bfloat16* dvp_lo, float* dA_acc, float* dtr_acc,
                      bool after_lbs, cudaStream_t st) {
  if (m.ntv == 0) return 0;
  const int groups = Sw / 32;
  const int pitch = m.vt_maxcols | 1;
  const size_t smem = joints_smem(JTL, pitch);
  B200_SMEM_ATTR_ONCE(joints_bwd_kernel, smem);
  LaunchTimer _timer("joints_bwd", st);
  B200_CUDA_TRY(launch_k(joints_bwd_kernel, dim3(groups, joints_split(m.ntv)), dim3(JT), smem, st, after_lbs, m,
                         reinterpret_cast<const float4*>(vpB), m.n_pad / 4, reinterpret_cast<const float4*>(A_blk), b0, nb, pitch,
                         dJ, dvp_hi, dvp_lo, dA_acc, dtr_acc));
  B200_LAUNCH_CHECK("joints_bwd");
  return 0;
}

int launch_joint_grad_total(const float* joints, const float* cam, const float* gj, const float* g2d, float* dJ,
                            float* gcam, int B, int nj, cudaStream_t st) {
  LaunchTimer _timer("joint_grad_total", st);
  joint_grad_total_kernel<<<B, 128, 0, st>>>(joints, cam, gj, g2d, dJ, gcam, nj);
  B200_LAUNCH_CHECK("joint_grad_total");
  return 0;
}

}
```

### soccerplayershapepose_b200/csrc/umma_common.cuh

```cuda
#pragma once

#include <cuda.h>

#include "skin_common.cuh"

namespace b200smpl {

constexpr int BM = 128;
constexpr int BK = 64;
constexpr int UMMA_K = 16;
constexpr int GEMM_THREADS = 192;

struct GemmOps {
  const __nv_bfloat16* dvp_hi;
  const __nv_bfloat16* dvp_lo;
  CUtensorMap wb_hi, wb_lo;
};

__device__ __forceinline__ uint32_t smem_u32(const void* p) { return (uint32_t)__cvta_generic_to_shared(p); }

__device__ __forceinline__ void mbar_arrive_expect_tx(uint64_t* bar, uint32_t bytes) {
  asm volatile("mbarrier.arrive.expect_tx.shared::cta.b64 _, [%0], %1;" ::"r"(smem_u32(bar)), "r"(bytes) : "memory");
}
__device__ __forceinline__ void fence_barrier_init() { asm volatile("fence.mbarrier_init.release.cluster;" ::: "memory"); }
__device__ __forceinline__ void fence_proxy_async() { asm volatile("fence.proxy.async.shared::cta;" ::: "memory"); }
__device__ __forceinline__ void tc_fence_before() { asm volatile("tcgen05.fence::before_thread_sync;" ::: "memory"); }
__device__ __forceinline__ void tc_fence_after() { asm volatile("tcgen05.fence::after_thread_sync;" ::: "memory"); }

__device__ __forceinline__ void tma_load_2d(void* smem_dst, const CUtensorMap* map, uint64_t* bar, int c0, int c1) {
  asm volatile(
      "cp.async.bulk.tensor.2d.shared::cluster.global.mbarrier::complete_tx::bytes [%0], [%1, {%3, %4}], [%2];"
      ::"r"(smem_u32(smem_dst)), "l"(map), "r"(smem_u32(bar)), "r"(c0), "r"(c1)
      : "memory");
}
__device__ __forceinline__ bool elect_one() {
  uint32_t pred;
  asm volatile(
      "{\n\t.reg .pred p;\n\t"
      "elect.sync _|p, 0xffffffff;\n\t"
      "selp.u32 %0, 1, 0, p;\n\t}"
      : "=r"(pred));
  return pred != 0;
}
__device__ __forceinline__ uint64_t l2_policy_evict_first() {
  uint64_t p;
  asm volatile("createpolicy.fractional.L2::evict_first.b64 %0, 1.0;" : "=l"(p));
  return p;
}
__device__ __forceinline__ uint64_t l2_policy_evict_last() {
  uint64_t p;
  asm volatile("createpolicy.fractional.L2::evict_last.b64 %0, 1.0;" : "=l"(p));
  return p;
}
__device__ __forceinline__ void tma_load_2d_hint(void* smem_dst, const CUtensorMap* map, uint64_t* bar, int c0, int c1,
                                                 uint64_t policy) {
  asm volatile(
      "cp.async.bulk.tensor.2d.shared::cluster.global.mbarrier::complete_tx::bytes.L2::cache_hint [%0], [%1, {%3, %4}], [%2], %5;"
      ::"r"(smem_u32(smem_dst)), "l"(map), "r"(smem_u32(bar)), "r"(c0), "r"(c1), "l"(policy)
      : "memory");
}
__device__ __forceinline__ void bulk_g2s_hint(void* smem_dst, const void* src, uint32_t bytes, uint64_t* bar, uint64_t policy) {
  asm volatile("cp.async.bulk.shared::cluster.global.mbarrier::complete_tx::bytes.L2::cache_hint [%0], [%1], %2, [%3], %4;"
               ::"r"(smem_u32(smem_dst)), "l"(src), "r"(bytes), "r"(smem_u32(bar)), "l"(policy)
               : "memory");
}
__device__ __forceinline__ uint32_t cluster_ctarank() {
  uint32_t r;
  asm volatile("mov.u32 %0, %%cluster_ctarank;" : "=r"(r));
  return r;
}
__device__ __forceinline__ void cluster_sync_all() {
  asm volatile("barrier.cluster.arrive.release.aligned;" ::: "memory");
  asm volatile("barrier.cluster.wait.acquire.aligned;" ::: "memory");
}
__device__ __forceinline__ void prefetch_tmap(const CUtensorMap* map) {
  asm volatile("prefetch.tensormap [%0];" ::"l"(map) : "memory");
}

__device__ __forceinline__ void tmem_ld_32x32(uint32_t taddr, uint32_t (&v)[32]) {
  asm volatile(
      "tcgen05.ld.sync.aligned.32x32b.x32.b32 "
      "{%0, %1, %2, %3, %4, %5, %6, %7, %8, %9, %10, %11, %12, %13, %14, %15, "
      "%16, %17, %18, %19, %20, %21, %22, %23, %24, %25, %26, %27, %28, %29, %30, %31}, [%32];"
      : "=r"(v[0]), "=r"(v[1]), "=r"(v[2]), "=r"(v[3]), "=r"(v[4]), "=r"(v[5]), "=r"(v[6]), "=r"(v[7]), "=r"(v[8]),
        "=r"(v[9]), "=r"(v[10]), "=r"(v[11]), "=r"(v[12]), "=r"(v[13]), "=r"(v[14]), "=r"(v[15]), "=r"(v[16]),
        "=r"(v[17]), "=r"(v[18]), "=r"(v[19]), "=r"(v[20]), "=r"(v[21]), "=r"(v[22]), "=r"(v[23]), "=r"(v[24]),
        "=r"(v[25]), "=r"(v[26]), "=r"(v[27]), "=r"(v[28]), "=r"(v[29]), "=r"(v[30]), "=r"(v[31])
      : "r"(taddr)
      : "memory");
  asm volatile("tcgen05.wait::ld.sync.aligned;" ::: "memory");
}

__device__ __forceinline__ uint64_t make_sw128_desc(uint32_t smem_addr) {
  return (uint64_t)((smem_addr & 0x3FFFFu) >> 4) | (1ull << 16) | ((uint64_t)(1024 >> 4) << 32) | (1ull << 46) |
         (2ull << 61);
}

__device__ __forceinline__ uint64_t make_nosw_desc(uint32_t smem_addr, uint32_t lbo, uint32_t sbo) {
  return (uint64_t)((smem_addr & 0x3FFFFu) >> 4) | ((uint64_t)(lbo >> 4) << 16) | ((uint64_t)(sbo >> 4) << 32) |
         (1ull << 46);
}

__host__ __device__ constexpr uint32_t make_idesc(int M, int N) {
  return (1u << 4) | (1u << 7) | (1u << 10) | ((uint32_t)(N >> 3) << 17) | ((uint32_t)(M >> 4) << 24);
}

__device__ __forceinline__ void umma_bf16_2cta(uint32_t tmem_d, uint64_t desc_a, uint64_t desc_b, uint32_t idesc,
                                               uint32_t accumulate) {
  asm volatile(
      "{\n\t.reg .pred p;\n\t"
      "setp.ne.b32 p, %4, 0;\n\t"
      "tcgen05.mma.cta_group::2.kind::f16 [%0], %1, %2, %3, p;\n\t}"
      ::"r"(tmem_d), "l"(desc_a), "l"(desc_b), "r"(idesc), "r"(accumulate)
      : "memory");
}
__device__ __forceinline__ void umma_commit_2cta(uint64_t* bar) {
  asm volatile("tcgen05.commit.cta_group::2.mbarrier::arrive::one.shared::cluster.multicast::cluster.b64 [%0], %1;"
               ::"r"(smem_u32(bar)), "h"((uint16_t)3)
               : "memory");
}
__device__ __forceinline__ void remote_arrive(uint64_t* local_bar, uint32_t cta) {
  uint32_t remote;
  asm volatile("mapa.shared::cluster.u32 %0, %1, %2;" : "=r"(remote) : "r"(smem_u32(local_bar)), "r"(cta));
  asm volatile("mbarrier.arrive.relaxed.cluster.shared::cluster.b64 _, [%0];" ::"r"(remote) : "memory");
}

constexpr int BS_MAX_WORK = 160;
struct BsWork {
  uint16_t bp[BS_MAX_WORK], w0[BS_MAX_WORK], w1[BS_MAX_WORK];
};
int build_bs_work(int bp_total, int wtp_total, int tpcs, BsWork& work);
int make_map(CUtensorMap* map, const void* base, int k_extent, int rows, int pitch_elems, int box_rows);

}
```

Baseline: 6.939 million.

## Load pose-segment tails as 16-column swizzle-32 tiles and fuse saved-path forward

Result: faster. 7.091 million (median of 6 runs) (+2.2%).

```diff
diff --git a/soccerplayershapepose_b200/csrc/api.cu b/soccerplayershapepose_b200/csrc/api.cu
--- a/soccerplayershapepose_b200/csrc/api.cu
+++ b/soccerplayershapepose_b200/csrc/api.cu
@@ -317,10 +317,10 @@
     }
     if ((rc = launch_pose_fwd(d, a->betas, a->pose, aa, b0, nb, S, Sw, feat, featf, A_T, a->transl, a->joints, st)))
       return rc;
-    const bool fused = a->vertices != nullptr && a->mode != B200SMPL_MODE_FP32_SIMT && saved == nullptr && nb >= 512;
+    const bool fused = a->vertices != nullptr && a->mode != B200SMPL_MODE_FP32_SIMT && nb >= 512;
     if (fused) {
-      rc = launch_blend_lbs_fwd(d, fwd_gemm_mode(a->mode), feat, S, Sw, vpT, A_T, b0, nb, a->transl, a->vertices,
-                                m->num_sms, st);
+      rc = launch_blend_lbs_fwd(d, fwd_gemm_mode(a->mode), feat, S, Sw, vpT, saved != nullptr, A_T, b0, nb, a->transl,
+                                a->vertices, m->num_sms, st);
     } else if (a->mode == B200SMPL_MODE_FP32_SIMT) {
       rc = launch_blend_fwd_simt(d, featf, S, Sw, vpT, row_begin, d.n_pad, st);
     } else {
@@ -329,7 +329,8 @@
     if (rc) return rc;
     if (a->vertices && !fused)
       if ((rc = launch_lbs_fwd(d, vpT, S, A_T, b0, nb, a->transl, a->vertices, m->num_sms, st))) return rc;
-    if ((rc = launch_joints_fwd(d, vpT, S, A_T, b0, nb, a->transl, a->joints, a->vertices != nullptr && !fused, st))) return rc;
+    if ((rc = launch_joints_fwd(d, vpT, S, A_T, b0, nb, a->transl, a->joints, a->vertices != nullptr && !fused, fused, st)))
+      return rc;
   }
   if (a->joints2d)
     if ((rc = b200smpl_orthographic_project(a->joints, a->cam, a->joints2d, B, d.njout, 0.f, stream))) return rc;
diff --git a/soccerplayershapepose_b200/csrc/blend_umma.cu b/soccerplayershapepose_b200/csrc/blend_umma.cu
--- a/soccerplayershapepose_b200/csrc/blend_umma.cu
+++ b/soccerplayershapepose_b200/csrc/blend_umma.cu
@@ -150,24 +150,30 @@
 }
 
 constexpr int WS_STAGES = 5;
-constexpr int WS_MAX_SLABS = 9;
+constexpr int WS_PS = (NPOSE + BK - 1) / BK;
+constexpr int WS_PF = POSE_FULL_SLABS;
+constexpr int WS_MAX_SLABS = 1 + 2 * WS_PF;
 constexpr int WS_BN = 128;
+constexpr int WS_TAIL = WS_BN * POSE_TAIL_COLS * 2;
+static_assert(WS_PS == WS_PF + 1, "a pose segment is its full slabs and one tail tile");
 
 
 template <int DUMMY>
 __global__ void __launch_bounds__(GEMM_THREADS, 1)
-blend_fwd_bs2_kernel(const __grid_constant__ CUtensorMap map_w, const __grid_constant__ CUtensorMap map_f, int pslabs,
-                     int ksteps_cs, int ksteps_p, int use_lo, int row0, int mtiles, int ntiles_n,
+blend_fwd_bs2_kernel(const __grid_constant__ CUtensorMap map_w, const __grid_constant__ CUtensorMap map_f,
+                     const __grid_constant__ CUtensorMap map_wt, const __grid_constant__ CUtensorMap map_ft,
+                     int ksteps_cs, int use_lo, int row0, int mtiles, int ntiles_n,
                      const __grid_constant__ BsWork work, float4* __restrict__ vpB, int nc4) {
   constexpr int SLAB = BM * BK * 2;
   constexpr int KS = BK / UMMA_K;
   constexpr uint32_t TMEM_COLS = 512;
-  const int nslab_f = 1 + 2 * pslabs;
-  const int nslab_w = 1 + (use_lo ? 2 : 1) * pslabs;
+  constexpr int PS = WS_PS, PF = WS_PF;
+  const int nslab_w = 1 + (use_lo ? 2 : 1) * PS;
   extern __shared__ unsigned char smem_dyn[];
   unsigned char* smem = reinterpret_cast<unsigned char*>((reinterpret_cast<uintptr_t>(smem_dyn) + 1023) & ~(uintptr_t)1023);
   unsigned char* f_s = smem;
-  unsigned char* w_s = smem + WS_MAX_SLABS * SLAB;
+  unsigned char* ft_s = f_s + WS_MAX_SLABS * SLAB;
+  unsigned char* w_s = ft_s + 2 * WS_TAIL;
   uint64_t* bars = reinterpret_cast<uint64_t*>(w_s + WS_STAGES * SLAB);
   uint64_t* f_full = bars;
   uint64_t* peer_f_full = bars + 1;
@@ -187,6 +193,8 @@
   if (warp == 0 && lane == 0) {
     prefetch_tmap(&map_w);
     prefetch_tmap(&map_f);
+    prefetch_tmap(&map_wt);
+    prefetch_tmap(&map_ft);
   }
   if (warp == 1 && lane == 0) {
     mbar_init(f_full, 1);
@@ -217,8 +225,13 @@
 
   if (warp == 0) {
     if (elect_one()) {
-      mbar_arrive_expect_tx(f_full, (uint32_t)nslab_f * SLAB);
-      for (int s = 0; s < nslab_f; ++s) tma_load_2d(f_s + s * SLAB, &map_f, f_full, s * BK, btile * WS_BN);
+      mbar_arrive_expect_tx(f_full, WS_MAX_SLABS * SLAB + 2 * WS_TAIL);
+      tma_load_2d(f_s, &map_f, f_full, 0, btile * WS_BN);
+      for (int seg = 0; seg < 2; ++seg) {
+        for (int j = 0; j < PF; ++j)
+          tma_load_2d(f_s + (1 + seg * PF + j) * SLAB, &map_f, f_full, (1 + seg * PS + j) * BK, btile * WS_BN);
+        tma_load_2d(ft_s + seg * WS_TAIL, &map_ft, f_full, (1 + seg * PS + PF) * BK, btile * WS_BN);
+      }
     }
     __syncwarp();
     const uint64_t pol_keep = l2_policy_evict_last();
@@ -228,8 +241,10 @@
       for (int s = 0; s < nslab_w; ++s) {
         mbar_wait(&empty_bar[stage], phase ^ 1);
         if (elect_one()) {
-          mbar_arrive_expect_tx(&full_bar[stage], SLAB);
-          tma_load_2d_hint(w_s + stage * SLAB, &map_w, &full_bar[stage], s * BK, row0 + (wtp * 2 + (int)rank) * BM, pol_keep);
+          const bool tail = s > 0 && (s - 1) % PS == PF;
+          mbar_arrive_expect_tx(&full_bar[stage], tail ? WS_TAIL : SLAB);
+          tma_load_2d_hint(w_s + stage * SLAB, tail ? &map_wt : &map_w, &full_bar[stage], s * BK,
+                           row0 + (wtp * 2 + (int)rank) * BM, pol_keep);
         }
         __syncwarp();
         if (++stage == WS_STAGES) { stage = 0; phase ^= 1; }
@@ -253,21 +268,24 @@
           mbar_wait(&full_bar[stage], phase);
           mbar_wait(&peer_full_bar[stage], phase);
           tc_fence_after();
-          const uint64_t db = make_sw128_desc(smem_u32(w_s + stage * SLAB));
-          int ks = ksteps_cs, f0 = 0, f1 = -1;
-          if (s > 0) {
-            const int j = (s - 1) % pslabs;
-            ks = min(KS, ksteps_p - j * KS);
-            f0 = 1 + j;
-            if (s <= pslabs) f1 = 1 + pslabs + j;
+          const int j = s > 0 ? (s - 1) % PS : 0;
+          const bool tail = s > 0 && j == PF, with_lo = s > 0 && s <= PS;
+          const int ks = s == 0 ? ksteps_cs : tail ? 1 : KS;
+          uint64_t db, da0, da1;
+          if (tail) {
+            db = make_sw32_desc(smem_u32(w_s + stage * SLAB));
+            da0 = make_sw32_desc(smem_u32(ft_s));
+            da1 = make_sw32_desc(smem_u32(ft_s + WS_TAIL));
+          } else {
+            db = make_sw128_desc(smem_u32(w_s + stage * SLAB));
+            da0 = make_sw128_desc(smem_u32(f_s + (s == 0 ? 0 : 1 + j) * SLAB));
+            da1 = make_sw128_desc(smem_u32(f_s + (1 + PF + j) * SLAB));
           }
-          const uint64_t da0 = make_sw128_desc(smem_u32(f_s + f0 * SLAB));
-          const uint64_t da1 = make_sw128_desc(smem_u32(f_s + max(f1, 0) * SLAB));
           if (elect_one()) {
 #pragma unroll
             for (int k = 0; k < KS; ++k)
               if (k < ks) umma_bf16_2cta(d_tmem, da0 + 2 * k, db + 2 * k, idesc, (s | k) != 0);
-            if (f1 >= 0) {
+            if (with_lo) {
 #pragma unroll
               for (int k = 0; k < KS; ++k)
                 if (k < ks) umma_bf16_2cta(d_tmem, da1 + 2 * k, db + 2 * k, idesc, 1u);
@@ -347,18 +365,26 @@
   return fn;
 }
 
-int make_map(CUtensorMap* map, const void* base, int k_extent, int rows, int pitch_elems, int box_rows) {
+static int encode_map(CUtensorMap* map, const void* base, int k_extent, int rows, int pitch_elems, int box_k,
+                      int box_rows, CUtensorMapSwizzle swizzle) {
   EncodeTiledFn fn = get_encode_fn();
   if (fn == nullptr) return fail(B200SMPL_ERR_CUDA, "cuTensorMapEncodeTiled entry point not available");
   cuuint64_t dims[2] = {(cuuint64_t)k_extent, (cuuint64_t)rows};
   cuuint64_t strides[1] = {(cuuint64_t)pitch_elems * 2};
-  cuuint32_t box[2] = {(cuuint32_t)BK, (cuuint32_t)box_rows};
+  cuuint32_t box[2] = {(cuuint32_t)box_k, (cuuint32_t)box_rows};
   cuuint32_t estr[2] = {1, 1};
   CUresult r = fn(map, CU_TENSOR_MAP_DATA_TYPE_BFLOAT16, 2, const_cast<void*>(base), dims, strides, box, estr,
-                  CU_TENSOR_MAP_INTERLEAVE_NONE, CU_TENSOR_MAP_SWIZZLE_128B, CU_TENSOR_MAP_L2_PROMOTION_L2_256B,
+                  CU_TENSOR_MAP_INTERLEAVE_NONE, swizzle, CU_TENSOR_MAP_L2_PROMOTION_L2_256B,
                   CU_TENSOR_MAP_FLOAT_OOB_FILL_NONE);
   if (r != CUDA_SUCCESS) return fail(B200SMPL_ERR_CUDA, "cuTensorMapEncodeTiled failed with code " + std::to_string((int)r));
   return 0;
+}
+
+int make_map(CUtensorMap* map, const void* base, int k_extent, int rows, int pitch_elems, int box_rows) {
+  return encode_map(map, base, k_extent, rows, pitch_elems, BK, box_rows, CU_TENSOR_MAP_SWIZZLE_128B);
+}
+int make_map_tail(CUtensorMap* map, const void* base, int k_extent, int rows, int pitch_elems, int box_rows) {
+  return encode_map(map, base, k_extent, rows, pitch_elems, POSE_TAIL_COLS, box_rows, CU_TENSOR_MAP_SWIZZLE_32B);
 }
 
 int build_bs_work(int bp_total, int wtp_total, int tpcs, BsWork& work) {
@@ -399,14 +425,16 @@
 
 int launch_blend_fwd_umma(const DevModel& m, int mode, const __nv_bfloat16* feat, int S, int Sw, float* vpT,
                           int row_begin, int row_end, int num_sms, cudaStream_t st) {
-  const int pslabs = m.fl.pseg / BK;
   const int use_lo = (mode == B200SMPL_MODE_BF16) ? 0 : 1;
-  if (1 + 2 * pslabs > WS_MAX_SLABS) return fail(B200SMPL_ERR_INVALID, "feature pitch too large for the resident operand");
-  CUtensorMap map_w, map_f;
+  if (m.fl.pseg != WS_PS * BK) return fail(B200SMPL_ERR_INVALID, "forward GEMM: unexpected pose segment width");
+  CUtensorMap map_w, map_f, map_wt, map_ft;
   int rc;
   if ((rc = make_map(&map_w, m.Wf, m.fl.pitch, m.n_pad, m.fl.pitch, BM))) return rc;
   if ((rc = make_map(&map_f, feat, m.fl.pitch, Sw, m.fl.pitch, WS_BN))) return rc;
-  constexpr int smem = (WS_MAX_SLABS + WS_STAGES) * BM * BK * 2 + 1024 + 256;
+  if ((rc = make_map_tail(&map_wt, m.Wf, m.fl.pitch, m.n_pad, m.fl.pitch, BM))) return rc;
+  if ((rc = make_map_tail(&map_ft, feat, m.fl.pitch, Sw, m.fl.pitch, WS_BN))) return rc;
+  constexpr int smem = (WS_MAX_SLABS + WS_STAGES) * BM * BK * 2 + 2 * WS_TAIL + 1024 + 256;
+  static_assert(smem <= 232448, "forward GEMM: shared memory budget");
   auto kern = blend_fwd_bs2_kernel<0>;
   B200_SMEM_ATTR_ONCE(kern, smem);
   const int mtiles = (row_end - row_begin) / BM;
@@ -432,9 +460,8 @@
   cfg.attrs = attr;
   cfg.numAttrs = pdl_enabled() ? 2 : 1;
   LaunchTimer _timer("blend_fwd_umma", st);
-  B200_CUDA_TRY(cudaLaunchKernelEx(&cfg, kern, map_w, map_f, pslabs, (m.fl.k_cs + UMMA_K - 1) / UMMA_K,
-                                   (NPOSE + UMMA_K - 1) / UMMA_K, use_lo, row_begin, mtiles, ntiles_n, work,
-                                   reinterpret_cast<float4*>(vpT), m.n_pad / 4));
+  B200_CUDA_TRY(cudaLaunchKernelEx(&cfg, kern, map_w, map_f, map_wt, map_ft, (m.fl.k_cs + UMMA_K - 1) / UMMA_K, use_lo,
+                                   row_begin, mtiles, ntiles_n, work, reinterpret_cast<float4*>(vpT), m.n_pad / 4));
   B200_LAUNCH_CHECK("blend_fwd_umma");
   return 0;
 }
diff --git a/soccerplayershapepose_b200/csrc/common.cuh b/soccerplayershapepose_b200/csrc/common.cuh
--- a/soccerplayershapepose_b200/csrc/common.cuh
+++ b/soccerplayershapepose_b200/csrc/common.cuh
@@ -210,7 +210,7 @@
                           int S, int Sw, float* dfeat_part, int nsplit, int row_begin, int row_end,
                           cudaStream_t st);
 int blend_bwd_umma_splits(const DevModel& m, int S, int num_sms);
-int launch_blend_lbs_fwd(const DevModel& m, int mode, const __nv_bfloat16* feat, int S, int Sw, float* vpT,
+int launch_blend_lbs_fwd(const DevModel& m, int mode, const __nv_bfloat16* feat, int S, int Sw, float* vpT, int write_vp,
                          const float* A_blk, int b0, int nb, const float* transl, float* verts, int num_sms,
                          cudaStream_t st);
 
@@ -221,7 +221,7 @@
                    float* dtr_acc, int num_sms, cudaStream_t st);
 
 int launch_joints_fwd(const DevModel& m, const float* vpB, int S, const float* A_blk, int b0, int nb,
-                      const float* transl, float* joints, bool after_lbs, cudaStream_t st);
+                      const float* transl, float* joints, bool after_lbs, bool after_fused, cudaStream_t st);
 int launch_joints_bwd(const DevModel& m, const float* vpB, int S, int Sw, const float* A_blk, int b0, int nb,
                       const float* dJ, __nv_bfloat16* dvp_hi, __nv_bfloat16* dvp_lo, float* dA_part, float* dtr_part,
                       bool after_lbs, cudaStream_t st);
diff --git a/soccerplayershapepose_b200/csrc/fused_fwd.cu b/soccerplayershapepose_b200/csrc/fused_fwd.cu
--- a/soccerplayershapepose_b200/csrc/fused_fwd.cu
+++ b/soccerplayershapepose_b200/csrc/fused_fwd.cu
@@ -8,12 +8,14 @@
 constexpr int FF_BN = 96;
 constexpr int FF_BNH = FF_BN / 2;
 constexpr int FF_NW = 2;
-constexpr int FF_STAGES = 7;
+constexpr int FF_STAGES = 11;
 constexpr int FF_STAGE_BYTES = FF_BNH * BK * 2;
 constexpr int FF_PS = (NPOSE + BK - 1) / BK;
-constexpr int FF_KSP = (NPOSE + UMMA_K - 1) / UMMA_K;
-constexpr int FF_MAX_SLABS = 1 + 2 * FF_PS;
+constexpr int FF_PF = POSE_FULL_SLABS;
+constexpr int FF_MAX_SLABS = 1 + 2 * FF_PF;
 constexpr int FF_SLAB = BM * BK * 2;
+constexpr int FF_FTAIL = BM * POSE_TAIL_COLS * 2;
+constexpr int FF_WTAIL = FF_BNH * POSE_TAIL_COLS * 2;
 constexpr int FF_EPI_WARPS = 4 * FF_NW;
 constexpr int FF_EPI_WARP0 = 2;
 constexpr int FF_THREADS = (FF_EPI_WARP0 + FF_EPI_WARPS) * 32;
@@ -23,10 +25,13 @@
 constexpr int FF_PLAN_WORDS = (FF_WV / 8) * 40;
 constexpr int FF_TILE_WORDS = ItemShape<FF_HV>::TILE_WORDS;
 constexpr int FF_NBARS = 1 + 2 * FF_STAGES + 4 + 2 * FF_EPI_WARPS;
-constexpr size_t FF_SMEM = (size_t)FF_MAX_SLABS * FF_SLAB + (size_t)FF_STAGES * FF_STAGE_BYTES +
+constexpr size_t FF_SMEM = (size_t)FF_MAX_SLABS * FF_SLAB + 2 * FF_FTAIL + (size_t)FF_STAGES * FF_STAGE_BYTES +
                            (size_t)FF_EPI_WARPS * (FF_TILE_WORDS + 2 * FF_PLAN_WORDS) * 4 + FF_NBARS * 8 + 16 +
                            1024 ;
 static_assert(FF_SMEM <= 232448, "fused forward: shared memory budget");
+static_assert((FF_MAX_SLABS * FF_SLAB + 2 * FF_FTAIL) % 1024 == 0 && FF_STAGE_BYTES % 1024 == 0,
+              "swizzled tiles start on 1024-byte boundaries");
+static_assert(FF_PS == FF_PF + 1, "a pose segment is its full slabs and one tail tile");
 static_assert(FF_TR_COL + NJ * AELEMS <= 512, "fused forward: tensor memory budget");
 static_assert(NJ % FF_NW == 0, "joints split evenly over the warps of a quadrant");
 
@@ -123,20 +128,22 @@
 template <bool USE_LO>
 __global__ void __launch_bounds__(FF_THREADS, 1)
 blend_lbs_fwd_kernel(const __grid_constant__ CUtensorMap map_w, const __grid_constant__ CUtensorMap map_f,
+                     const __grid_constant__ CUtensorMap map_wt, const __grid_constant__ CUtensorMap map_ft,
                      int ksteps_cs, int n_pad, int ntiles_n,
-                     const __grid_constant__ BsWork work, float4* __restrict__ vpB, int nc4,
+                     const __grid_constant__ BsWork work, float4* __restrict__ vpB, int nc4, int write_vp,
                      const float4* __restrict__ A_blk, int b0, int nb, const float* __restrict__ transl,
                      float* __restrict__ verts, int V, int n_vtiles, int vec_ok, const uint32_t* __restrict__ vplan) {
   constexpr int KS = BK / UMMA_K;
   constexpr uint32_t TMEM_COLS = 512;
   using SH = ItemShape<FF_HV>;
   constexpr int PS = FF_PS;
-  constexpr int nslab_f = 1 + 2 * PS;
+  constexpr int PF = FF_PF;
   constexpr int nslab_w = 1 + (USE_LO ? 2 : 1) * PS;
   extern __shared__ __align__(1024) unsigned char smem_dyn[];
   unsigned char* smem = smem_dyn + ((1024u - (smem_u32(smem_dyn) & 1023u)) & 1023u);
   unsigned char* f_s = smem;
-  unsigned char* w_s = f_s + FF_MAX_SLABS * FF_SLAB;
+  unsigned char* ft_s = f_s + FF_MAX_SLABS * FF_SLAB;
+  unsigned char* w_s = ft_s + 2 * FF_FTAIL;
   float* tiles = reinterpret_cast<float*>(w_s + FF_STAGES * FF_STAGE_BYTES);
   uint32_t* stashes = reinterpret_cast<uint32_t*>(tiles + FF_EPI_WARPS * FF_TILE_WORDS);
   uint64_t* bars = reinterpret_cast<uint64_t*>(stashes + FF_EPI_WARPS * 2 * FF_PLAN_WORDS);
@@ -157,6 +164,8 @@
   if (warp == 0 && lane == 0) {
     prefetch_tmap(&map_w);
     prefetch_tmap(&map_f);
+    prefetch_tmap(&map_wt);
+    prefetch_tmap(&map_ft);
   }
   if (warp == 1 && lane == 0) {
     mbar_init(f_full, 1);
@@ -188,8 +197,14 @@
   if (warp == 0) {
     const uint64_t pol_keep = l2_policy_evict_last();
     if (elect_one()) {
-      if (rank == 0) mbar_arrive_expect_tx(f_full, 2u * (uint32_t)nslab_f * FF_SLAB);
-      for (int s = 0; s < nslab_f; ++s) tma_load_2d_pair(f_s + s * FF_SLAB, &map_f, f_full, s * BK, btile * BM, l2_policy_evict_first());
+      const uint64_t pol_once = l2_policy_evict_first();
+      if (rank == 0) mbar_arrive_expect_tx(f_full, 2u * (FF_MAX_SLABS * FF_SLAB + 2 * FF_FTAIL));
+      tma_load_2d_pair(f_s, &map_f, f_full, 0, btile * BM, pol_once);
+      for (int seg = 0; seg < 2; ++seg) {
+        for (int j = 0; j < PF; ++j)
+          tma_load_2d_pair(f_s + (1 + seg * PF + j) * FF_SLAB, &map_f, f_full, (1 + seg * PS + j) * BK, btile * BM, pol_once);
+        tma_load_2d_pair(ft_s + seg * FF_FTAIL, &map_ft, f_full, (1 + seg * PS + PF) * BK, btile * BM, pol_once);
+      }
     }
     __syncwarp();
     int stage = 0;
@@ -198,8 +213,10 @@
       for (int s = 0; s < nslab_w; ++s) {
         mbar_wait(&empty_bar[stage], phase ^ 1);
         if (elect_one()) {
-          if (rank == 0) mbar_arrive_expect_tx(&full_bar[stage], 2 * FF_STAGE_BYTES);
-          tma_load_2d_pair(w_s + stage * FF_STAGE_BYTES, &map_w, &full_bar[stage], s * BK, wt * FF_BN + (int)rank * FF_BNH, pol_keep);
+          const bool tail = s > 0 && (s - 1) % PS == PF;
+          if (rank == 0) mbar_arrive_expect_tx(&full_bar[stage], 2 * (tail ? FF_WTAIL : FF_STAGE_BYTES));
+          tma_load_2d_pair(w_s + stage * FF_STAGE_BYTES, tail ? &map_wt : &map_w, &full_bar[stage], s * BK,
+                           wt * FF_BN + (int)rank * FF_BNH, pol_keep);
         }
         __syncwarp();
         if (++stage == FF_STAGES) { stage = 0; phase ^= 1; }
@@ -212,6 +229,8 @@
       mbar_wait(f_full, 0);
       const uint64_t da_base = make_sw128_desc(smem_u32(f_s));
       const uint64_t db_base = make_sw128_desc(smem_u32(w_s));
+      const uint64_t dat_hi = make_sw32_desc(smem_u32(ft_s)), dat_lo = make_sw32_desc(smem_u32(ft_s + FF_FTAIL));
+      const uint64_t dbt_base = make_sw32_desc(smem_u32(w_s));
       uint32_t tph0 = 0, tph1 = 0;
       int acc = 0;
       auto slab = [&](uint32_t d_tmem, int ks, int f0, int f1, bool first, uint64_t* tfull) {
@@ -229,6 +248,19 @@
             for (int k = 0; k < KS; ++k)
               if (k < ks) umma_bf16_2cta(d_tmem, da1 + 2 * k, db + 2 * k, idesc, 1u);
           }
+          umma_commit_2cta(&empty_bar[stage]);
+          if (tfull != nullptr) umma_commit_2cta(tfull);
+        }
+        __syncwarp();
+        if (++stage == FF_STAGES) { stage = 0; phase ^= 1; }
+      };
+      auto tail = [&](uint32_t d_tmem, bool with_lo, uint64_t* tfull) {
+        mbar_wait(&full_bar[stage], phase);
+        tc_fence_after();
+        const uint64_t db = dbt_base + (uint64_t)(stage * (FF_STAGE_BYTES >> 4));
+        if (elect_one()) {
+          umma_bf16_2cta(d_tmem, dat_hi, db, idesc, 1u);
+          if (with_lo) umma_bf16_2cta(d_tmem, dat_lo, db, idesc, 1u);
           umma_commit_2cta(&empty_bar[stage]);
           if (tfull != nullptr) umma_commit_2cta(tfull);
         }
@@ -244,12 +276,12 @@
         const uint32_t d_tmem = tmem_base + (uint32_t)(acc * FF_BN);
         slab(d_tmem, ksteps_cs, 0, -1, true, nullptr);
 #pragma unroll
-        for (int j = 0; j < PS; ++j)
-          slab(d_tmem, min(KS, FF_KSP - j * KS), 1 + j, 1 + PS + j, false, (!USE_LO && j == PS - 1) ? &tfull_bar[acc] : nullptr);
+        for (int j = 0; j < PF; ++j) slab(d_tmem, KS, 1 + j, 1 + PF + j, false, nullptr);
+        tail(d_tmem, true, USE_LO ? nullptr : &tfull_bar[acc]);
         if (USE_LO) {
 #pragma unroll
-          for (int j = 0; j < PS; ++j)
-            slab(d_tmem, min(KS, FF_KSP - j * KS), 1 + j, -1, false, j == PS - 1 ? &tfull_bar[acc] : nullptr);
+          for (int j = 0; j < PF; ++j) slab(d_tmem, KS, 1 + j, -1, false, nullptr);
+          tail(d_tmem, false, &tfull_bar[acc]);
         }
       }
     }
@@ -319,6 +351,7 @@
       }
       const int row_w = wt * FF_BN + half * (FF_BN / 2);
       const uint32_t acc_base = lane_base + (uint32_t)(acc * FF_BN + half * (FF_BN / 2));
+      float4* colbase = vpB + ((size_t)g * nc4 + (row_w >> 2)) * 32 + lane;
       if (skin && wt < n_vtiles) {
         const uint32_t b = n_plan & 1;
         if (is_vhalf(h + FF_NW) && lane == 0) issue_plan(b ^ 1, h + FF_NW);
@@ -329,6 +362,12 @@
           uint32_t v[24];
           tmem_ld_24(acc_base + (uint32_t)(sub * 24), v);
           if (sub == FF_WV / FF_HV - 1) release(acc);
+          if (write_vp) {
+#pragma unroll
+            for (int i = 0; i < 6; ++i)
+              colbase[(size_t)(sub * 6 + i) * 32] = make_float4(__uint_as_float(v[4 * i]), __uint_as_float(v[4 * i + 1]),
+                                                                __uint_as_float(v[4 * i + 2]), __uint_as_float(v[4 * i + 3]));
+          }
 #pragma unroll
           for (int u = 0; u < FF_HV / 4; ++u) {
             float P[12];
@@ -350,7 +389,6 @@
         }
         ++n_plan;
       } else {
-        float4* colbase = vpB + ((size_t)g * nc4 + (row_w >> 2)) * 32 + lane;
 #pragma unroll 1
         for (int c0 = 0; c0 < FF_BN / 2; c0 += 24) {
           uint32_t v[24];
@@ -374,17 +412,19 @@
   }
 }
 
-int launch_blend_lbs_fwd(const DevModel& m, int mode, const __nv_bfloat16* feat, int S, int Sw, float* vpT,
+int launch_blend_lbs_fwd(const DevModel& m, int mode, const __nv_bfloat16* feat, int S, int Sw, float* vpT, int write_vp,
                          const float* A_blk, int b0, int nb, const float* transl, float* verts, int num_sms,
                          cudaStream_t st) {
   (void)S;
   const bool use_lo = mode != B200SMPL_MODE_BF16;
   if (m.fl.pseg != FF_PS * BK) return fail(B200SMPL_ERR_INVALID, "fused forward: unexpected pose segment width");
   if (m.n_virt0 != m.ntiles * FF_BN) return fail(B200SMPL_ERR_INVALID, "fused forward: vertex tiles must be 96 rows");
-  CUtensorMap map_w, map_f;
+  CUtensorMap map_w, map_f, map_wt, map_ft;
   int rc;
   if ((rc = make_map(&map_w, m.Wf, m.fl.pitch, m.n_pad, m.fl.pitch, FF_BNH))) return rc;
   if ((rc = make_map(&map_f, feat, m.fl.pitch, Sw, m.fl.pitch, BM))) return rc;
+  if ((rc = make_map_tail(&map_wt, m.Wf, m.fl.pitch, m.n_pad, m.fl.pitch, FF_BNH))) return rc;
+  if ((rc = make_map_tail(&map_ft, feat, m.fl.pitch, Sw, m.fl.pitch, BM))) return rc;
   auto kern = use_lo ? blend_lbs_fwd_kernel<true> : blend_lbs_fwd_kernel<false>;
   B200_SMEM_ATTR_ONCE(blend_lbs_fwd_kernel<true>, FF_SMEM);
   B200_SMEM_ATTR_ONCE(blend_lbs_fwd_kernel<false>, FF_SMEM);
@@ -411,8 +451,9 @@
   cfg.attrs = attr;
   cfg.numAttrs = pdl_enabled() ? 2 : 1;
   LaunchTimer _timer("blend_lbs_fwd", st);
-  B200_CUDA_TRY(cudaLaunchKernelEx(&cfg, kern, map_w, map_f, (m.fl.k_cs + UMMA_K - 1) / UMMA_K, m.n_pad, ntiles_n, work,
-                                   reinterpret_cast<float4*>(vpT), m.n_pad / 4, reinterpret_cast<const float4*>(A_blk), b0, nb,
+  B200_CUDA_TRY(cudaLaunchKernelEx(&cfg, kern, map_w, map_f, map_wt, map_ft, (m.fl.k_cs + UMMA_K - 1) / UMMA_K, m.n_pad,
+                                   ntiles_n, work, reinterpret_cast<float4*>(vpT), m.n_pad / 4, write_vp,
+                                   reinterpret_cast<const float4*>(A_blk), b0, nb,
                                    transl, verts, m.V, m.ntiles, vec_ok, m.vplan));
   B200_LAUNCH_CHECK("blend_lbs_fwd");
   return 0;
diff --git a/soccerplayershapepose_b200/csrc/joints.cu b/soccerplayershapepose_b200/csrc/joints.cu
--- a/soccerplayershapepose_b200/csrc/joints.cu
+++ b/soccerplayershapepose_b200/csrc/joints.cu
@@ -22,7 +22,8 @@
 
 __global__ void __launch_bounds__(JT, 1024 / JT)
 joints_fwd_kernel(DevModel m, const float4* __restrict__ vpB, int nc4, const float4* __restrict__ A_blk, int b0, int nb,
-                  int pitch, const float* __restrict__ transl, float* __restrict__ joints) {
+                  int pitch, const float* __restrict__ transl, float* __restrict__ joints, int wait_first) {
+  if (wait_first) pdl_wait();
   extern __shared__ __align__(128) float smem[];
   float* A_s = smem;
   const int warp = threadIdx.x >> 5, lane = threadIdx.x & 31;
@@ -203,16 +204,16 @@
 static size_t joints_smem(int ntiles_s, int pitch) { return (size_t)(AG_WORDS + ntiles_s * 32 * pitch + 1) * 4 + 16; }
 
 int launch_joints_fwd(const DevModel& m, const float* vpB, int S, const float* A_blk, int b0, int nb,
-                      const float* transl, float* joints, bool after_lbs, cudaStream_t st) {
+                      const float* transl, float* joints, bool after_lbs, bool after_fused, cudaStream_t st) {
   if (nb <= 0 || m.ntv == 0) return 0;
   const int groups = (nb + 31) / 32;
   const int pitch = m.vt_maxcols | 1;
   const size_t smem = joints_smem(JW, pitch);
   B200_SMEM_ATTR_ONCE(joints_fwd_kernel, smem);
   LaunchTimer _timer("joints_fwd", st);
-  B200_CUDA_TRY(launch_k(joints_fwd_kernel, dim3(groups, joints_split(m.ntv)), dim3(JT), smem, st, after_lbs, m,
-                         reinterpret_cast<const float4*>(vpB), m.n_pad / 4, reinterpret_cast<const float4*>(A_blk), b0, nb, pitch,
-                         transl, joints));
+  B200_CUDA_TRY(launch_k(joints_fwd_kernel, dim3(groups, joints_split(m.ntv)), dim3(JT), smem, st, after_lbs || after_fused,
+                         m, reinterpret_cast<const float4*>(vpB), m.n_pad / 4, reinterpret_cast<const float4*>(A_blk), b0, nb,
+                         pitch, transl, joints, after_fused ? 1 : 0));
   B200_LAUNCH_CHECK("joints_fwd");
   return 0;
 }
diff --git a/soccerplayershapepose_b200/csrc/umma_common.cuh b/soccerplayershapepose_b200/csrc/umma_common.cuh
--- a/soccerplayershapepose_b200/csrc/umma_common.cuh
+++ b/soccerplayershapepose_b200/csrc/umma_common.cuh
@@ -96,6 +96,11 @@
          (2ull << 61);
 }
 
+__device__ __forceinline__ uint64_t make_sw32_desc(uint32_t smem_addr) {
+  return (uint64_t)((smem_addr & 0x3FFFFu) >> 4) | (1ull << 16) | ((uint64_t)(256 >> 4) << 32) | (1ull << 46) |
+         (6ull << 61);
+}
+
 __device__ __forceinline__ uint64_t make_nosw_desc(uint32_t smem_addr, uint32_t lbo, uint32_t sbo) {
   return (uint64_t)((smem_addr & 0x3FFFFu) >> 4) | ((uint64_t)(lbo >> 4) << 16) | ((uint64_t)(sbo >> 4) << 32) |
          (1ull << 46);
@@ -131,5 +136,11 @@
 };
 int build_bs_work(int bp_total, int wtp_total, int tpcs, BsWork& work);
 int make_map(CUtensorMap* map, const void* base, int k_extent, int rows, int pitch_elems, int box_rows);
+int make_map_tail(CUtensorMap* map, const void* base, int k_extent, int rows, int pitch_elems, int box_rows);
+
+constexpr int POSE_FULL_SLABS = NPOSE / BK;
+constexpr int POSE_TAIL_COLS = UMMA_K;
+static_assert(POSE_FULL_SLABS * BK < NPOSE && NPOSE <= POSE_FULL_SLABS * BK + POSE_TAIL_COLS,
+              "a pose segment is full 64-column slabs plus one 16-column K step");
 
 }
```
